# lastdancewithyou/multimodal_edema_prediction

Hardware: AMD Instinct MI355X
Metric: multimodal train samples/sec (higher is better)
Workload: dtype bf16

## Files before the change

### include/medp_hip.h

```cpp
#ifndef MEDP_HIP_H
#define MEDP_HIP_H
#include <stddef.h>

#ifdef __cplusplus
extern "C" {
#endif

const char* medp_last_error(void);
int medp_version(void);
const char* medp_arch(void);

int medp_gemm_bf16_nt(const void* A, const void* W, void* C, int M, int N, int K, int lda, int ldw, int ldc,
                      const float* bias, const float* scale, const float* residual, int ldr, int act, int out_bf16,
                      void* stream);

size_t medp_gemm_nt_workspace_bytes(int M, int N, int K);
int medp_gemm_bf16_nt_ws(const void* A, const void* W, void* C, int M, int N, int K, int lda, int ldw, int ldc, const float* bias,
                         const float* scale, const float* residual, int ldr, int act, int out_bf16, float* workspace,
                         size_t workspace_bytes, void* stream);

int medp_gemm_f32_nt(const float* A, const float* W, float* C, int M, int N, int K, int lda, int ldw, int ldc, const float* bias,
                     const float* scale, const float* residual, int ldr, int act, void* stream);
int medp_gemm_f32_tn(const float* dY, const float* X, float* C, int M, int N, int K, int lddy, int ldx, void* stream);

size_t medp_gemm_tn_workspace_bytes(int M, int N, int K);
int medp_gemm_bf16_tn(const void* dY, const void* X, float* C, int M, int N, int K, int lddy, int ldx, float* workspace, void* stream);

int medp_gemm_persistent_cap(int cap);

int medp_gemm_profile_enable(int mode);
int medp_gemm_profile_collect(double* host_total_ms, long long* host_n_launches, double* host_total_flops);

int medp_attn_fwd_dh64(const void* q, const void* k, const void* v, void* o, int B, int S, int H, int ldq, int ldk,
                       int ldv, int ldo, float scale, void* stream);
int medp_attn_dh16_fwd(const float* qkv, int ld, void* o_bf16, int ldo, int B, int N, int H, int dh, float scale, void* stream);
int medp_attn_dh16_train_supported(int B, int N, int H, int dh, int ld, int ldo);
int medp_attn_dh16_train_fwd(const void* qkv, int ld, void* o, int ldo, float* lse, int io_bf16, int B, int N, int H, int dh, float scale,
                             float dropout_p, unsigned seed, unsigned stream_id, void* stream);
int medp_attn_dh16_train_bwd(const void* dout, int lddo, const void* qkv, int ld, const float* lse, float* delta_ws, void* dqkv,
                             int lddqkv, int io_bf16, int B, int N, int H, int dh, float scale, float dropout_p, unsigned seed,
                             unsigned stream_id, void* stream);
int medp_attn_fwd_dh64_lse(const void* q, const void* k, const void* v, void* o, float* lse, int B, int S, int H, int ldq,
                           int ldk, int ldv, int ldo, float scale, void* stream);
int medp_attn_bwd_dh64_prep(const float* dout, int lddout, const void* o_bf16, int ldo, void* dout_bf16, int lddob,
                            float* dsum, int B, int S, int H, void* stream);
int medp_attn_bwd_dh64(const void* q, const void* k, const void* v, int ldqkv, const void* dout_bf16, int lddo,
                       const float* lse, const float* dsum, float* dq, float* dk, float* dv, int ldd, int B, int S, int H,
                       float scale, void* stream);
int medp_attn_small_fwd(const float* q, int ldq, long long q_batch_stride, const float* k, const float* v, int ldkv,
                        long long kv_batch_stride, void* o, int ldo, int o_bf16, float* attn_avg, int B, int Lq, int Lk,
                        int H, int dh, float scale, float dropout_p, unsigned seed, unsigned stream_id, void* stream);
int medp_attn_small_bwd(const float* dout, int lddo, const float* q, int ldq, long long q_batch_stride, const float* k,
                        const float* v, int ldkv, long long kv_batch_stride, float* dq, int lddq, float* dk, int lddkv,
                        float* dv, int reserved, long long dkv_batch_stride, int B, int Lq, int Lk, int H, int dh, float scale,
                        float dropout_p, unsigned seed, unsigned stream_id, void* stream);
int medp_attn_small_masked_fwd(const float* q, int ldq, long long q_batch_stride, const float* k, const float* v, int ldkv,
                               long long kv_batch_stride, void* o, int ldo, int o_bf16, float* attn_avg, int B, int Lq, int Lk,
                               int H, int dh, float scale, float dropout_p, unsigned seed, unsigned stream_id, void* stream,
                               const unsigned char* key_mask, long long mask_batch_stride);
int medp_attn_small_masked_bwd(const float* dout, int lddo, const float* q, int ldq, long long q_batch_stride, const float* k,
                               const float* v, int ldkv, long long kv_batch_stride, float* dq, int lddq, float* dk, int lddkv,
                               float* dv, int reserved, long long dkv_batch_stride, int B, int Lq, int Lk, int H, int dh, float scale,
                               float dropout_p, unsigned seed, unsigned stream_id, void* stream, const unsigned char* key_mask,
                               long long mask_batch_stride);

size_t medp_attn_fq_split_ws_bytes(int B, int H, int Lq, int Lk, int bwd);
int medp_attn_fq_split_fwd(const float* q, int ldq, long long q_batch_stride, const float* k, const float* v, int ldkv,
                           long long kv_batch_stride, void* o, int ldo, int o_bf16, float* lse, float* attn_avg, float* ws,
                           size_t ws_bytes, int B, int Lq, int Lk, int H, int dh, float scale, float dropout_p, unsigned seed,
                           unsigned stream_id, void* stream);
int medp_attn_fq_split_bwd(const float* dout, int lddo, const float* o, int ldo, const float* lse, const float* q, int ldq,
                           long long q_batch_stride, const float* k, const float* v, int ldkv, long long kv_batch_stride, float* dq,
                           int lddq, float* dk, float* dv, int lddkv, long long dkv_batch_stride, float* ws, size_t ws_bytes, int B,
                           int Lq, int Lk, int H, int dh, float scale, float dropout_p, unsigned seed, unsigned stream_id,
                           void* stream);

int medp_layernorm_fwd(const float* x, int ldx, const float* w, const float* b, void* y, int ldy, int y_bf16, float* mean,
                       float* rstd, int rows, int D, float eps, void* stream);
size_t medp_colsum_workspace_bytes(int rows, int D);
int medp_layernorm_bwd(const float* dy, int lddy, const float* x, int ldx, const float* w, const float* mean,
                       const float* rstd, float* dx, int lddx, int accumulate_dx, float* dw, float* db, float* workspace,
                       int rows, int D, void* stream);
int medp_colsum_f32(const float* x, int ldx, float* out, float* workspace, int rows, int D, void* stream);
int medp_scalenorm_fwd(const float* x, int ldx, const float* g, void* y, int ldy, int y_bf16, float* rnorm, int rows, int D,
                       float eps, void* stream);
int medp_scalenorm_bwd(const float* dy, int lddy, const float* x, int ldx, const float* g, const float* rnorm, float* dx,
                       int lddx, int accumulate_dx, float* dg, float* workspace_rows, int rows, int D, void* stream);
int medp_scalenorm_bwd_add(const float* dy, int lddy, const float* x, int ldx, const float* g, const float* rnorm, const float* add,
                           int ldadd, float* dx, int lddx, float* dg, float* workspace_rows, int rows, int D, void* stream);

int medp_cast_f32_bf16(const float* x, int ldx, void* y, int ldy, int rows, int cols, void* stream);
int medp_transpose_to_bf16(const void* x, int x_is_bf16, int ldx, void* y, int ldy, int rows, int cols, void* stream);
typedef struct {
    const void* src;
    void* dst_plain;
    void* dst_t;
    int rows, cols, ld_src, ld_plain, ld_t, reserved_;
} MedpOperandJob;
int medp_weight_operands_multi(const MedpOperandJob* dev_jobs, const int* dev_block_job, const int* dev_block_tile, int n_blocks,
                               void* stream);
int medp_gelu_bwd(const float* dy, const float* pre, float* dx, long long n, void* stream);
int medp_gelu_bf16_fwd(const void* pre, void* out, long long n, void* stream);
int medp_gelu_bf16_bwd(const void* dy, const void* pre, void* dx, long long n, void* stream);
int medp_im2col_patch(const float* pix, void* A, int B, int C, int H, int W, int patch, int kpad, void* stream);
int medp_vit_assemble(const float* patch, const float* cls, const float* pos, float* x, int B, int P, int D, void* stream);
int medp_pos_embed_bicubic(const float* pos, float* out, int src_side, int gh, int gw, int D, void* stream);
int medp_pos_embed_bicubic_bwd(const float* dout, float* dpos, int src_side, int gh, int gw, int D, void* stream);

typedef struct {
    const float *ln1_w, *ln1_b;
    const void* qkv_w;
    const float* qkv_b;
    const void* proj_w;
    const float *proj_b, *ls1;
    const float *ln2_w, *ln2_b;
    const void* fc1_w;
    const float* fc1_b;
    const void* fc2_w;
    const float *fc2_b, *ls2;
    const void *qkv_wg, *fc1_wg;
    const float *qkv_cs, *qkv_b2, *fc1_cs, *fc1_b2;
} MedpVitLayer;

typedef struct {
    int hidden, n_layers, n_heads, mlp_hidden, patch, pos_side, patch_kpad;
    float ln_eps;
    const void* patch_w;
    const float *patch_b, *cls, *pos;
    const float *final_ln_w, *final_ln_b;
    const MedpVitLayer* layers;
} MedpVitWeights;

size_t medp_vit_workspace_bytes(const MedpVitWeights* host_w, int B, int H, int W);
int medp_vit_forward(const MedpVitWeights* host_w, const float* pixels, int B, int H, int W, float* tokens_f32,
                     void* tokens_bf16, void* workspace, size_t workspace_bytes, void* stream);
int medp_vit_forward_part(const MedpVitWeights* w, const float* pixels, int B, int H, int W, float* tokens_f32, void* tokens_bf16,
                          void* workspace, size_t workspace_bytes, int first_layer, int last_layer, void* stream);

typedef struct {
    const float* g_attn;
    const void* qkv_w;
    const void* out_w;
    const float* g_ff;
    const void* ff1_w;
    const float* ff1_b;
    const void* ff2_w;
    const float* ff2_b;
    const float* g_final;
} MedpEncoderWeights;

typedef struct {
    int n_vars, n_static, d_embedding, n_heads, n_layers, d_ff, d_hidden_embed, d_hidden_tab, d_hidden_time, n_obs_rows,
        final_norm;
    float norm_eps;
    const void *emb_w0, *emb_b0, *emb_bn_scale, *emb_bn_shift, *emb_w4, *emb_b4;
    const void *emb_l0, *emb_w4t;
    const void* n_obs_table;
    const void *tab_w0, *tab_b0, *tab_bn_scale, *tab_bn_shift, *tab_w4, *tab_b4;
    const void* special;
    const void *time_w0, *time_b0, *time_bn_scale, *time_bn_shift, *time_w3t, *time_b3;
    const void* rep_embedding;
    const void* event_embedding;
    const MedpEncoderWeights* event_enc;
    const MedpEncoderWeights* time_enc;
} MedpDuettWeights;

int medp_duett_embed_fwd(const MedpDuettWeights* host_w, const float* xs_static, const float* xs_ts, const float* xs_times, int B, int T,
                         float* xe_out, void* h_out_bf16, float* temb_out, float* psi0_out, float* tab_workspace, int stages, void* stream);
int medp_duett_swap_add_norm(const float* in, const float* rnorm, const float* g_prev, const float* add, long long add_batch_stride,
                             const float* g_norm, float norm_eps, float* x_out, void* h_out_bf16, int B, int A1, int A2, int E,
                             void* stream);

int medp_feats_to_input(const float* const* ts_ptrs, const float* ts_base, long long ts_stride, const float* const* time_ptrs,
                        const float* time_base, long long time_stride, const int* lengths, int T_uniform, const float* static_in,
                        float* xs_ts, float* xs_times, float* xs_static, int B, int V, int Ds, int max_len, int Tpad, float aug_noise,
                        float aug_mask, unsigned seed, unsigned stream_id, void* stream);
int medp_ssl_mask_batch(const float* xs_ts, const int* mask_t, const int* event_idx, const unsigned char* keep, float* clipped,
                        float* y_ts, float* y_masks, float* y_events, float* y_events_mask, int B, int T, int V, void* stream);

size_t medp_duett_workspace_bytes(const MedpDuettWeights* host_w, int B, int T);
int medp_duett_encode(const MedpDuettWeights* host_w, const float* xs_static, const float* xs_ts, const float* xs_times, int B,
                      int T, float* tokens_f32, void* tokens_bf16, float* psi0_out, void* workspace, size_t workspace_bytes,
                      void* stream);

int medp_gelu_dropout_fwd(const float* x, float* y, long long n, float p, unsigned seed, unsigned stream_id, void* stream);
int medp_gelu_dropout_bwd(const float* dy, const float* x, float* dx, long long n, float p, unsigned seed, unsigned stream_id,
                          void* stream);
int medp_gelu_dropout_fwd_bf16(const float* x, void* y_bf16, long long n, float p, unsigned seed, unsigned stream_id, void* stream);
int medp_gelu_dropout_bwd_bf16(const float* dy, const float* x, float* dx, void* dx_bf16, long long n, float p, unsigned seed,
                               unsigned stream_id, void* stream);
int medp_dropout_add(const float* y, const float* residual, float* out, long long n, float p, unsigned seed, unsigned stream_id,
                     void* stream);
int medp_rowdot_fwd(const float* x, int ldx, const float* w, const float* b, float* y, int rows, int D, void* stream);
int medp_rowdot_bwd(const float* dy, const float* x, int ldx, const float* w, float* dx, float* dw, float* db, int rows, int D,
                    void* stream);
int medp_fusion_logits_fwd(const float* hi, const float* ht, const float* hc, const float* img_bias, const float* ts_bias,
                           const float* beta, float* img, float* ts, float* scaled, float* fus, int B, int K, void* stream);
int medp_fusion_logits_bwd(const float* d_img, const float* d_ts, const float* d_scaled, const float* d_fus, const float* hc,
                           const float* beta, float* d_hi, float* d_ht, float* d_hc, float* d_img_bias, float* d_ts_bias,
                           float* d_beta, int B, int K, void* stream);
int medp_meanpool_fwd(const float* x, float* y, int B, int T, int T1, int D, void* stream);
int medp_meanpool_bwd(const float* dy, float* dx, int B, int T, int T1, int D, void* stream);

int medp_dual_pathology_loss(const float* img, const float* ts, const float* fus, const float* y, const float* mask,
                             const float* label_weights, const float* pos_weight, float alpha_img, float alpha_ts,
                             float alpha_fus, float eps, float* out, float* g_img, float* g_ts, float* g_fus, int B, int K,
                             void* stream);
int medp_student_kd_loss(const float* z_s, const float* z_t, const float* y, float T, float alpha, float pos_weight, float* out,
                         float* g_zs, int B, void* stream);

int medp_aux_residual_kl(const float* img_logits, const float* scaled_correction, const float* y, const float* mask,
                         float label_smoothing, float* out, float* g_scaled, int n, void* stream);
int medp_sq_mean(const float* x, float coef, float* out, float* g, int n, void* stream);
int medp_masked_bce_global(const float* logits, const float* y, const float* mask, float* out, float* g, int n, void* stream);

int medp_masked_mse(const float* a, const float* b, const float* mask, float* out, float* g_a, int n, void* stream);
int medp_bce_mean(const float* logits, const float* y, const float* weight, float* out, float* g, int n, void* stream);

typedef struct {
    void* param;
    const void* grad;
    void* exp_avg;
    void* exp_avg_sq;
    long long numel;
    float lr, weight_decay;
} MedpAdamTensor;
int medp_adamw_chunk_elems(void);
int medp_adamw_multi(const MedpAdamTensor* dev_descs, const int* dev_block_tensor, const int* dev_block_chunk, int n_blocks,
                     float beta1, float beta2, float eps, int step, const unsigned* dev_step, float grad_scale, void* stream);
int medp_grad_sumsq_multi(const MedpAdamTensor* dev_descs, const int* dev_block_tensor, const int* dev_block_chunk, int n_blocks,
                          float* dev_partials, float max_norm, float* dev_out, void* stream);
int medp_adamw_multi_dscale(const MedpAdamTensor* dev_descs, const int* dev_block_tensor, const int* dev_block_chunk, int n_blocks,
                            float beta1, float beta2, float eps, int step, const unsigned* dev_step, const float* dev_grad_scale,
                            void* stream);

int medp_rng_set_epoch_ptr(const unsigned* dev_ptr);
int medp_counter_advance(unsigned* dev_counter, void* stream);

int medp_glinear_fwd(const float* x, const float* W, const float* b, float* y, int G, int R, int K, int N, void* stream);
size_t medp_glinear_bwd_workspace_bytes(int G, int R, int K, int N);
int medp_glinear_bwd(const float* dy, const float* x, const float* W, float* dx, float* dW, float* db, float* workspace, int G, int R,
                     int K, int N, void* stream);
int medp_gmlp_supported(int KIN, int C, int E);
size_t medp_gmlp_workspace_bytes(int G, int R, int KIN, int C, int E);
int medp_gmlp_fwd(const float* x, const float* W0, const float* b0, const float* bn_w, const float* bn_b, float* running_mean,
                  float* running_var, const float* W1, const float* b1, float* out, float* save_mean, float* save_var, int G, int R,
                  int KIN, int C, int E, float eps, float momentum, int batch_stats, float* workspace, void* stream);
int medp_gmlp_bwd(const float* dout, const float* x, const float* W0, const float* b0, const float* bn_w, const float* bn_b,
                  const float* save_mean, const float* save_var, const float* W1, float* dx, float* dW0, float* db0, float* dbn_w,
                  float* dbn_b, float* dW1, float* db1, int G, int R, int KIN, int C, int E, float eps, int batch_stats,
                  float* workspace, void* stream);
size_t medp_gbn_workspace_bytes(int G, int R, int C);
int medp_gbn_fwd(const float* x, const float* w, const float* b, float* running_mean, float* running_var, float* y, float* save_mean,
                 float* save_var, int G, int R, int C, float eps, float momentum, int batch_stats, float* workspace, void* stream);
int medp_gbn_bwd(const float* dy, const float* x, const float* w, const float* save_mean, const float* save_var, float* dx, float* dw,
                 float* db, int G, int R, int C, float eps, int batch_stats, float* workspace, void* stream);
int medp_act_fwd(const float* x, float* y, long long n, int mode , void* stream);
int medp_act_bwd(const float* dy, const float* y, float* dx, long long n, int mode, void* stream);
int medp_embed_inputs_fwd(const float* xs_ts, const float* n_obs_table, int table_rows, float* xin, int B, int T, int V, int KP,
                          void* stream);
int medp_embed_inputs_bwd_blocks(int B, int T, int V);
int medp_embed_inputs_bwd(const float* xs_ts, const float* d_xin, float* partial, int table_rows, int B, int T, int V, int KP,
                          void* stream);
int medp_psi_assemble_fwd(const float* xs_ts, const float* var_out, const float* tab_out, const float* special, float* psi, int B, int T,
                          int V, int E, void* stream);
int medp_psi_assemble_bwd_slices(int B, int T, int V);
int medp_psi_assemble_bwd(const float* xs_ts, const float* dpsi, float* d_var_out, float* d_tab_partial, float* d_special_partial, int B,
                          int T, int V, int E, void* stream);
int medp_axis_swap(const float* in, float* out, int B, int A1, int A2, int E, void* stream);
int medp_axis_swap_add(const float* in, const float* add, const float* add_last, float* out, int B, int A1, int A2, int E, int mode,
                       void* stream);
int medp_add_bcast(const float* a, const float* b, float* out, long long per_batch, int B, int broadcast_b, void* stream);

int medp_traj_features(const float* x, float* out, int B, int T, int V, void* stream);
int medp_gru_fwd(const float* gi, const void* whh_bf16, const float* bhh, float* hseq, float* gates, float* hn, int S, int T, int d,
                 void* stream);
int medp_gru_fwd_f32(const float* gi, const float* whh_t, int ld_whh_t, const float* bhh, float* hseq, float* gates, float* hn, int S,
                     int T, int d, void* stream);
int medp_gru_bwd(const float* dh, const float* gates, const float* hn, const float* hseq, const void* whh_t_bf16, float* dgi,
                 float* dghn, void* dgh_bf16, int S, int T, int d, void* stream);

#ifdef __cplusplus
}
#endif
#endif
```

### multimodal_edema_prediction_amd/abi.py

```python
from __future__ import annotations

import ctypes
import os
from ctypes import c_char_p, c_float, c_int, c_longlong, c_size_t, c_uint, c_void_p

import torch

_HERE = os.path.dirname(os.path.abspath(__file__))
LIB_PATH = os.environ.get("MEDP_HIP_LIB") or os.path.join(_HERE, "libmedp_hip.so")

P, I, F, U, LL, SZ = c_void_p, c_int, c_float, c_uint, c_longlong, c_size_t


class MedpVitLayer(ctypes.Structure):
    _fields_ = [(n, P) for n in ("ln1_w", "ln1_b", "qkv_w", "qkv_b", "proj_w", "proj_b", "ls1", "ln2_w", "ln2_b",
                                 "fc1_w", "fc1_b", "fc2_w", "fc2_b", "ls2",
                                 "qkv_wg", "fc1_wg", "qkv_cs", "qkv_b2", "fc1_cs", "fc1_b2")]


class MedpVitWeights(ctypes.Structure):
    _fields_ = ([(n, I) for n in ("hidden", "n_layers", "n_heads", "mlp_hidden", "patch", "pos_side", "patch_kpad")]
                + [("ln_eps", F)]
                + [(n, P) for n in ("patch_w", "patch_b", "cls", "pos", "final_ln_w", "final_ln_b")]
                + [("layers", ctypes.POINTER(MedpVitLayer))])


class MedpEncoderWeights(ctypes.Structure):
    _fields_ = [(n, P) for n in ("g_attn", "qkv_w", "out_w", "g_ff", "ff1_w", "ff1_b", "ff2_w", "ff2_b", "g_final")]


class MedpDuettWeights(ctypes.Structure):
    _fields_ = ([(n, I) for n in ("n_vars", "n_static", "d_embedding", "n_heads", "n_layers", "d_ff", "d_hidden_embed",
                                  "d_hidden_tab", "d_hidden_time", "n_obs_rows", "final_norm")]
                + [("norm_eps", F)]
                + [(n, P) for n in ("emb_w0", "emb_b0", "emb_bn_scale", "emb_bn_shift", "emb_w4", "emb_b4", "emb_l0", "emb_w4t", "n_obs_table",
                                    "tab_w0", "tab_b0", "tab_bn_scale", "tab_bn_shift", "tab_w4", "tab_b4", "special",
                                    "time_w0", "time_b0", "time_bn_scale", "time_bn_shift", "time_w3t", "time_b3",
                                    "rep_embedding", "event_embedding")]
                + [("event_enc", ctypes.POINTER(MedpEncoderWeights)), ("time_enc", ctypes.POINTER(MedpEncoderWeights))])


class MedpAdamTensor(ctypes.Structure):
    _fields_ = [("param", P), ("grad", P), ("exp_avg", P), ("exp_avg_sq", P), ("numel", LL), ("lr", F), ("weight_decay", F)]


class MedpOperandJob(ctypes.Structure):
    _fields_ = [("src", P), ("dst_plain", P), ("dst_t", P), ("rows", I), ("cols", I), ("ld_src", I), ("ld_plain", I), ("ld_t", I),
                ("reserved_", I)]


SIGNATURES = {
    "medp_last_error": (c_char_p, []),
    "medp_version": (I, []),
    "medp_arch": (c_char_p, []),
    "medp_gemm_bf16_nt": (I, [P, P, P, I, I, I, I, I, I, P, P, P, I, I, I, P]),
    "medp_gemm_nt_workspace_bytes": (SZ, [I, I, I]),
    "medp_gemm_bf16_nt_ws": (I, [P, P, P, I, I, I, I, I, I, P, P, P, I, I, I, P, SZ, P]),
    "medp_gemm_f32_nt": (I, [P, P, P, I, I, I, I, I, I, P, P, P, I, I, P]),
    "medp_gemm_f32_tn": (I, [P, P, P, I, I, I, I, I, P]),
    "medp_gemm_tn_workspace_bytes": (SZ, [I, I, I]),
    "medp_gemm_bf16_tn": (I, [P, P, P, I, I, I, I, I, P, P]),
    "medp_gemm_persistent_cap": (I, [I]),
    "medp_gemm_profile_enable": (I, [I]),
    "medp_gemm_profile_collect": (I, [ctypes.POINTER(ctypes.c_double), ctypes.POINTER(c_longlong), ctypes.POINTER(ctypes.c_double)]),
    "medp_attn_fwd_dh64": (I, [P, P, P, P, I, I, I, I, I, I, I, F, P]),
    "medp_attn_dh16_fwd": (I, [P, I, P, I, I, I, I, I, F, P]),
    "medp_attn_dh16_train_supported": (I, [I, I, I, I, I, I]),
    "medp_attn_dh16_train_fwd": (I, [P, I, P, I, P, I, I, I, I, I, F, F, U, U, P]),
    "medp_attn_dh16_train_bwd": (I, [P, I, P, I, P, P, P, I, I, I, I, I, I, F, F, U, U, P]),
    "medp_attn_fwd_dh64_lse": (I, [P, P, P, P, P, I, I, I, I, I, I, I, F, P]),
    "medp_attn_bwd_dh64_prep": (I, [P, I, P, I, P, I, P, I, I, I, P]),
    "medp_attn_bwd_dh64": (I, [P, P, P, I, P, I, P, P, P, P, P, I, I, I, I, F, P]),
    "medp_attn_small_fwd": (I, [P, I, LL, P, P, I, LL, P, I, I, P, I, I, I, I, I, F, F, U, U, P]),
    "medp_attn_small_bwd": (I, [P, I, P, I, LL, P, P, I, LL, P, I, P, I, P, I, LL, I, I, I, I, I, F, F, U, U, P]),
    "medp_attn_small_masked_fwd": (I, [P, I, LL, P, P, I, LL, P, I, I, P, I, I, I, I, I, F, F, U, U, P, P, LL]),
    "medp_attn_small_masked_bwd": (I, [P, I, P, I, LL, P, P, I, LL, P, I, P, I, P, I, LL, I, I, I, I, I, F, F, U, U, P, P, LL]),
    "medp_attn_fq_split_ws_bytes": (SZ, [I, I, I, I, I]),
    "medp_attn_fq_split_fwd": (I, [P, I, LL, P, P, I, LL, P, I, I, P, P, P, SZ, I, I, I, I, I, F, F, U, U, P]),
    "medp_attn_fq_split_bwd": (I, [P, I, P, I, P, P, I, LL, P, P, I, LL, P, I, P, P, I, LL, P, SZ, I, I, I, I, I, F, F, U, U, P]),
    "medp_layernorm_fwd": (I, [P, I, P, P, P, I, I, P, P, I, I, F, P]),
    "medp_colsum_workspace_bytes": (SZ, [I, I]),
    "medp_layernorm_bwd": (I, [P, I, P, I, P, P, P, P, I, I, P, P, P, I, I, P]),
    "medp_colsum_f32": (I, [P, I, P, P, I, I, P]),
    "medp_scalenorm_fwd": (I, [P, I, P, P, I, I, P, I, I, F, P]),
    "medp_scalenorm_bwd": (I, [P, I, P, I, P, P, P, I, I, P, P, I, I, P]),
    "medp_scalenorm_bwd_add": (I, [P, I, P, I, P, P, P, I, P, I, P, P, I, I, P]),
    "medp_cast_f32_bf16": (I, [P, I, P, I, I, I, P]),
    "medp_transpose_to_bf16": (I, [P, I, I, P, I, I, I, P]),
    "medp_weight_operands_multi": (I, [P, P, P, I, P]),
    "medp_gelu_bwd": (I, [P, P, P, LL, P]),
    "medp_gelu_bf16_fwd": (I, [P, P, LL, P]),
    "medp_gelu_bf16_bwd": (I, [P, P, P, LL, P]),
    "medp_im2col_patch": (I, [P, P, I, I, I, I, I, I, P]),
    "medp_vit_assemble": (I, [P, P, P, P, I, I, I, P]),
    "medp_pos_embed_bicubic": (I, [P, P, I, I, I, I, P]),
    "medp_pos_embed_bicubic_bwd": (I, [P, P, I, I, I, I, P]),
    "medp_vit_workspace_bytes": (SZ, [ctypes.POINTER(MedpVitWeights), I, I, I]),
    "medp_vit_forward": (I, [ctypes.POINTER(MedpVitWeights), P, I, I, I, P, P, P, SZ, P]),
    "medp_vit_forward_part": (I, [ctypes.POINTER(MedpVitWeights), P, I, I, I, P, P, P, SZ, I, I, P]),
    "medp_duett_embed_fwd": (I, [ctypes.POINTER(MedpDuettWeights), P, P, P, I, I, P, P, P, P, P, I, P]),
    "medp_duett_swap_add_norm": (I, [P, P, P, P, LL, P, F, P, P, I, I, I, I, P]),
    "medp_feats_to_input": (I, [P, P, LL, P, P, LL, P, I, P, P, P, P, I, I, I, I, I, F, F, U, U, P]),
    "medp_ssl_mask_batch": (I, [P, P, P, P, P, P, P, P, P, I, I, I, P]),
    "medp_duett_workspace_bytes": (SZ, [ctypes.POINTER(MedpDuettWeights), I, I]),
    "medp_duett_encode": (I, [ctypes.POINTER(MedpDuettWeights), P, P, P, I, I, P, P, P, P, SZ, P]),
    "medp_gelu_dropout_fwd": (I, [P, P, LL, F, U, U, P]),
    "medp_gelu_dropout_bwd": (I, [P, P, P, LL, F, U, U, P]),
    "medp_gelu_dropout_fwd_bf16": (I, [P, P, LL, F, U, U, P]),
    "medp_gelu_dropout_bwd_bf16": (I, [P, P, P, P, LL, F, U, U, P]),
    "medp_dropout_add": (I, [P, P, P, LL, F, U, U, P]),
    "medp_rowdot_fwd": (I, [P, I, P, P, P, I, I, P]),
    "medp_rowdot_bwd": (I, [P, P, I, P, P, P, P, I, I, P]),
    "medp_fusion_logits_fwd": (I, [P, P, P, P, P, P, P, P, P, P, I, I, P]),
    "medp_fusion_logits_bwd": (I, [P, P, P, P, P, P, P, P, P, P, P, P, I, I, P]),
    "medp_meanpool_fwd": (I, [P, P, I, I, I, I, P]),
    "medp_meanpool_bwd": (I, [P, P, I, I, I, I, P]),
    "medp_dual_pathology_loss": (I, [P, P, P, P, P, P, P, F, F, F, F, P, P, P, P, I, I, P]),
    "medp_student_kd_loss": (I, [P, P, P, F, F, F, P, P, I, P]),
    "medp_aux_residual_kl": (I, [P, P, P, P, F, P, P, I, P]),
    "medp_sq_mean": (I, [P, F, P, P, I, P]),
    "medp_masked_bce_global": (I, [P, P, P, P, P, I, P]),
    "medp_glinear_fwd": (I, [P, P, P, P, I, I, I, I, P]),
    "medp_glinear_bwd_workspace_bytes": (SZ, [I, I, I, I]),
    "medp_glinear_bwd": (I, [P, P, P, P, P, P, P, I, I, I, I, P]),
    "medp_gmlp_supported": (I, [I, I, I]),
    "medp_gmlp_workspace_bytes": (SZ, [I, I, I, I, I]),
    "medp_gmlp_fwd": (I, [P] * 12 + [I, I, I, I, I, F, F, I, P, P]),
    "medp_gmlp_bwd": (I, [P] * 16 + [I, I, I, I, I, F, I, P, P]),
    "medp_gbn_workspace_bytes": (SZ, [I, I, I]),
    "medp_gbn_fwd": (I, [P, P, P, P, P, P, P, P, I, I, I, F, F, I, P, P]),
    "medp_gbn_bwd": (I, [P, P, P, P, P, P, P, P, I, I, I, F, I, P, P]),
    "medp_act_fwd": (I, [P, P, LL, I, P]),
    "medp_act_bwd": (I, [P, P, P, LL, I, P]),
    "medp_embed_inputs_fwd": (I, [P, P, I, P, I, I, I, I, P]),
    "medp_embed_inputs_bwd_blocks": (I, [I, I, I]),
    "medp_embed_inputs_bwd": (I, [P, P, P, I, I, I, I, I, P]),
    "medp_psi_assemble_fwd": (I, [P, P, P, P, P, I, I, I, I, P]),
    "medp_psi_assemble_bwd_slices": (I, [I, I, I]),
    "medp_psi_assemble_bwd": (I, [P, P, P, P, P, I, I, I, I, P]),
    "medp_axis_swap": (I, [P, P, I, I, I, I, P]),
    "medp_axis_swap_add": (I, [P, P, P, P, I, I, I, I, I, P]),
    "medp_add_bcast": (I, [P, P, P, LL, I, I, P]),
    "medp_masked_mse": (I, [P, P, P, P, P, I, P]),
    "medp_bce_mean": (I, [P, P, P, P, P, I, P]),
    "medp_adamw_chunk_elems": (I, []),
    "medp_adamw_multi": (I, [P, P, P, I, F, F, F, I, P, F, P]),
    "medp_grad_sumsq_multi": (I, [P, P, P, I, P, F, P, P]),
    "medp_adamw_multi_dscale": (I, [P, P, P, I, F, F, F, I, P, P, P]),
    "medp_traj_features": (I, [P, P, I, I, I, P]),
    "medp_gru_fwd": (I, [P, P, P, P, P, P, I, I, I, P]),
    "medp_gru_fwd_f32": (I, [P, P, I, P, P, P, P, I, I, I, P]),
    "medp_gru_bwd": (I, [P, P, P, P, P, P, P, P, I, I, I, P]),
    "medp_rng_set_epoch_ptr": (I, [P]),
    "medp_counter_advance": (I, [P, P]),
}

_lib = None


def lib() -> ctypes.CDLL:
    global _lib
    if _lib is None:
        if not os.path.exists(LIB_PATH):
            raise RuntimeError(
                f"HIP extension {LIB_PATH} is missing: build it with `python -m multimodal_edema_prediction_amd.build` "
                "(hipcc --offload-arch=gfx950). There is no CPU fallback for the hot path.")
        L = ctypes.CDLL(LIB_PATH)
        for name, (res, args) in SIGNATURES.items():
            fn = getattr(L, name)
            fn.restype, fn.argtypes = res, args
        _lib = L
    return _lib


def check(rc: int, what: str = "") -> None:
    if rc == 0:
        return
    msg = lib().medp_last_error().decode("utf-8", "replace")
    if rc < 0:
        raise ValueError(f"{what}: {msg}" if what else msg)
    raise RuntimeError(f"{what}: HIP error {rc}: {msg}")


def stream() -> int:
    return torch.cuda.current_stream().cuda_stream


def ptr(t: torch.Tensor | None) -> int | None:
    if t is None:
        return None
    if not t.is_cuda:
        raise RuntimeError("libmedp_hip operates on GPU memory only (tensor is on %s); there is no CPU fallback" % t.device)
    return t.data_ptr()


def require_gpu() -> None:
    lib()
    if not torch.cuda.is_available():
        raise RuntimeError("no HIP device is visible: the MI355X hot path cannot run (there is no CPU fallback)")
```

### multimodal_edema_prediction_amd/csrc/api.cpp

```cpp
#include <stdarg.h>
#include <stdio.h>

#include "medp_hip.h"

static thread_local char g_err[512] = "";

void medp_set_error(const char* fmt, ...) {
    va_list ap;
    va_start(ap, fmt);
    vsnprintf(g_err, sizeof(g_err), fmt, ap);
    va_end(ap);
}

extern "C" const char* medp_last_error(void) { return g_err; }
extern "C" int medp_version(void) { return 2; }
extern "C" const char* medp_arch(void) { return "gfx950"; }

#include <stdint.h>
static const uint32_t* g_rng_epoch = nullptr;
const uint32_t* medp_rng_epoch_ptr() { return g_rng_epoch; }
extern "C" int medp_rng_set_epoch_ptr(const unsigned* dev_ptr) {
    g_rng_epoch = dev_ptr;
    return 0;
}
```

### multimodal_edema_prediction_amd/csrc/elementwise.hip

```cpp
#include "common.h"
#include "medp_hip.h"

namespace {

__global__ __launch_bounds__(256) void cast_f32_bf16_kernel(const float* __restrict__ x, int ldx, bf16_t* __restrict__ y, int ldy,
                                                            int rows, int cols) {
    const int c4 = cols >> 2;
    const size_t total = (size_t)rows * c4;
    for (size_t i = (size_t)blockIdx.x * 256 + threadIdx.x; i < total; i += (size_t)gridDim.x * 256) {
        const int r = (int)(i / c4), c = (int)(i % c4) * 4;
        const float4 v = *(const float4*)(x + (size_t)r * ldx + c);
        uint2 o;
        o.x = pack_bf2(v.x, v.y);
        o.y = pack_bf2(v.z, v.w);
        *(uint2*)(y + (size_t)r * ldy + c) = o;
    }
}

template <typename TIN>
__global__ __launch_bounds__(256) void transpose_to_bf16_kernel(const TIN* __restrict__ x, int ldx, bf16_t* __restrict__ y, int ldy,
                                                                int rows, int cols) {
    __shared__ float tile[64][65];
    const int r0 = blockIdx.y * 64, c0 = blockIdx.x * 64;
    const int tx = threadIdx.x & 63, ty = threadIdx.x >> 6;
    for (int i = ty; i < 64; i += 4) {
        const int r = r0 + i, c = c0 + tx;
        float v = 0.f;
        if (r < rows && c < cols) {
            if constexpr (sizeof(TIN) == 2) v = bf2f(((const bf16_t*)x)[(size_t)r * ldx + c]);
            else v = ((const float*)x)[(size_t)r * ldx + c];
        }
        tile[i][tx] = v;
    }
    __syncthreads();
    for (int i = ty; i < 64; i += 4) {
        const int c = c0 + i, r = r0 + tx;
        if (c < cols && r < rows) y[(size_t)c * ldy + r] = f2bf(tile[tx][i]);
    }
}

__global__ __launch_bounds__(256) void weight_operands_multi_kernel(const MedpOperandJob* __restrict__ jobs, const int* __restrict__ blk_job,
                                                                    const int* __restrict__ blk_tile) {
    __shared__ float tile[64][65];
    const MedpOperandJob j = jobs[blk_job[blockIdx.x]];
    const int tiles_c = (j.cols + 63) / 64;
    const int t = blk_tile[blockIdx.x];
    const int r0 = (t / tiles_c) * 64, c0 = (t % tiles_c) * 64;
    const int tx = threadIdx.x & 63, ty = threadIdx.x >> 6;
    const float* x = (const float*)j.src;
    bf16_t* yp = (bf16_t*)j.dst_plain;
    bf16_t* yt = (bf16_t*)j.dst_t;
    for (int i = ty; i < 64; i += 4) {
        const int r = r0 + i, c = c0 + tx;
        float v = 0.f;
        if (r < j.rows && c < j.cols) {
            v = x[(size_t)r * j.ld_src + c];
            if (yp) yp[(size_t)r * j.ld_plain + c] = f2bf(v);
        }
        tile[i][tx] = v;
    }
    if (!yt) return;
    __syncthreads();
    for (int i = ty; i < 64; i += 4) {
        const int c = c0 + i, r = r0 + tx;
        if (c < j.cols && r < j.rows) yt[(size_t)c * j.ld_t + r] = f2bf(tile[tx][i]);
    }
}

__global__ __launch_bounds__(256) void gelu_bwd_kernel(const float* __restrict__ dy, const float* __restrict__ pre, float* __restrict__ dx,
                                                       size_t n) {
    for (size_t i = ((size_t)blockIdx.x * 256 + threadIdx.x) * 4; i < n; i += (size_t)gridDim.x * 1024) {
        const float4 g = *(const float4*)(dy + i), p = *(const float4*)(pre + i);
        *(float4*)(dx + i) = make_float4(g.x * gelu_erf_grad(p.x), g.y * gelu_erf_grad(p.y), g.z * gelu_erf_grad(p.z),
                                         g.w * gelu_erf_grad(p.w));
    }
}

__global__ __launch_bounds__(256) void gelu_bf16_fwd_kernel(const bf16_t* __restrict__ pre, bf16_t* __restrict__ out, size_t n8) {
    for (size_t i = (size_t)blockIdx.x * 256 + threadIdx.x; i < n8; i += (size_t)gridDim.x * 256) {
        const uint4 p = *(const uint4*)(pre + i * 8);
        const uint32_t w[4] = {p.x, p.y, p.z, p.w};
        uint32_t o[4];
#pragma unroll
        for (int k = 0; k < 4; ++k) {
            const f32x2 g = gelu_erf2((f32x2){__uint_as_float(w[k] << 16), __uint_as_float(w[k] & 0xffff0000u)});
            o[k] = pack_bf2(g[0], g[1]);
        }
        *(uint4*)(out + i * 8) = make_uint4(o[0], o[1], o[2], o[3]);
    }
}
__global__ __launch_bounds__(256) void gelu_bf16_bwd_kernel(const bf16_t* __restrict__ dy, const bf16_t* __restrict__ pre,
                                                            bf16_t* __restrict__ dx, size_t n8) {
    for (size_t i = (size_t)blockIdx.x * 256 + threadIdx.x; i < n8; i += (size_t)gridDim.x * 256) {
        const uint4 g = *(const uint4*)(dy + i * 8), p = *(const uint4*)(pre + i * 8);
        const uint32_t gw[4] = {g.x, g.y, g.z, g.w}, pw[4] = {p.x, p.y, p.z, p.w};
        uint32_t o[4];
#pragma unroll
        for (int k = 0; k < 4; ++k) {
            const float a = __uint_as_float(gw[k] << 16) * gelu_erf_grad(__uint_as_float(pw[k] << 16));
            const float b = __uint_as_float(gw[k] & 0xffff0000u) * gelu_erf_grad(__uint_as_float(pw[k] & 0xffff0000u));
            o[k] = pack_bf2(a, b);
        }
        *(uint4*)(dx + i * 8) = make_uint4(o[0], o[1], o[2], o[3]);
    }
}

__global__ __launch_bounds__(256) void im2col_patch_kernel(const float* __restrict__ pix, bf16_t* __restrict__ A, int B, int C, int H,
                                                           int W, int ps, int kpad) {
    const unsigned gh = H / ps, gw = W / ps, K = C * ps * ps, pp = ps * ps, k8 = kpad >> 3;
    const unsigned total = (unsigned)B * gh * gw * k8;
    for (unsigned i = blockIdx.x * 256u + threadIdx.x; i < total; i += gridDim.x * 256u) {
        const unsigned kc = i % k8, row = i / k8;
        const unsigned px = row % gw, r2 = row / gw, py = r2 % gh, b = r2 / gh;
        const float* img = pix + (size_t)b * C * H * W + (size_t)(py * ps) * W + px * ps;
        float v[8];
#pragma unroll
        for (int u = 0; u < 8; ++u) {
            const unsigned kk = kc * 8 + u;
            float x = 0.f;
            if (kk < K) {
                const unsigned c = kk / pp, rem = kk - c * pp, ii = rem / ps, jj = rem - ii * ps;
                x = img[((size_t)c * H + ii) * W + jj];
            }
            v[u] = x;
        }
        uint4 o;
        o.x = pack_bf2(v[0], v[1]);
        o.y = pack_bf2(v[2], v[3]);
        o.z = pack_bf2(v[4], v[5]);
        o.w = pack_bf2(v[6], v[7]);
        *(uint4*)(A + (size_t)row * kpad + kc * 8) = o;
    }
}

__global__ __launch_bounds__(256) void vit_assemble_kernel(const float* __restrict__ patch, const float* __restrict__ cls,
                                                           const float* __restrict__ pos, float* __restrict__ x, int B, int P, int D) {
    const int d4 = D >> 2;
    const size_t total = (size_t)B * (P + 1) * d4;
    for (size_t i = (size_t)blockIdx.x * 256 + threadIdx.x; i < total; i += (size_t)gridDim.x * 256) {
        const int c = (int)(i % d4) * 4;
        const size_t tokrow = i / d4;
        const int t = (int)(tokrow % (P + 1)), b = (int)(tokrow / (P + 1));
        const float4 pe = *(const float4*)(pos + (size_t)t * D + c);
        const float4 v = (t == 0) ? *(const float4*)(cls + c) : *(const float4*)(patch + ((size_t)b * P + t - 1) * D + c);
        *(float4*)(x + tokrow * D + c) = make_float4(v.x + pe.x, v.y + pe.y, v.z + pe.z, v.w + pe.w);
    }
}

__device__ __forceinline__ float cubic1(float x, float A) { return ((A + 2.f) * x - (A + 3.f)) * x * x + 1.f; }
__device__ __forceinline__ float cubic2(float x, float A) { return ((A * x - 5.f * A) * x + 8.f * A) * x - 4.f * A; }
__global__ __launch_bounds__(256) void pos_bicubic_kernel(const float* __restrict__ pos, float* __restrict__ out, int s, int gh, int gw,
                                                          int D) {
    const size_t total = (size_t)(gh * gw + 1) * D;
    const float A = -0.75f;
    for (size_t i = (size_t)blockIdx.x * 256 + threadIdx.x; i < total; i += (size_t)gridDim.x * 256) {
        const int d = (int)(i % D), t = (int)(i / D);
        if (t == 0) { out[i] = pos[d]; continue; }
        const int oy = (t - 1) / gw, ox = (t - 1) % gw;
        const float sy = (float)s / (float)gh, sx = (float)s / (float)gw;
        const float fy = (oy + 0.5f) * sy - 0.5f, fx = (ox + 0.5f) * sx - 0.5f;
        const int iy = (int)floorf(fy), ix = (int)floorf(fx);
        const float ty = fy - iy, tx = fx - ix;
        const float wy[4] = {cubic2(ty + 1.f, A), cubic1(ty, A), cubic1(1.f - ty, A), cubic2(2.f - ty, A)};
        const float wx[4] = {cubic2(tx + 1.f, A), cubic1(tx, A), cubic1(1.f - tx, A), cubic2(2.f - tx, A)};
        float acc = 0.f;
#pragma unroll
        for (int a = 0; a < 4; ++a) {
            const int yy = min(max(iy - 1 + a, 0), s - 1);
            float rowacc = 0.f;
#pragma unroll
            for (int c = 0; c < 4; ++c) {
                const int xx = min(max(ix - 1 + c, 0), s - 1);
                rowacc += wx[c] * pos[(size_t)(1 + yy * s + xx) * D + d];
            }
            acc += wy[a] * rowacc;
        }
        out[i] = acc;
    }
}

__device__ __forceinline__ float bicubic_tap_weight(int src, int dst, int s, int g) {
    const float A = -0.75f;
    const float sc = (float)s / (float)g;
    const float f = (dst + 0.5f) * sc - 0.5f;
    const int i0 = (int)floorf(f);
    const float t = f - i0;
    const float w[4] = {cubic2(t + 1.f, A), cubic1(t, A), cubic1(1.f - t, A), cubic2(2.f - t, A)};
    float acc = 0.f;
#pragma unroll
    for (int a = 0; a < 4; ++a)
        if (min(max(i0 - 1 + a, 0), s - 1) == src) acc += w[a];
    return acc;
}
__global__ __launch_bounds__(256) void pos_bicubic_bwd_kernel(const float* __restrict__ dout, float* __restrict__ dpos, int s, int gh,
                                                              int gw, int D) {
    const int d4n = D >> 2;
    const int total = (s * s + 1) * d4n;
    for (int i = blockIdx.x * 256 + threadIdx.x; i < total; i += gridDim.x * 256) {
        const int d4 = i % d4n, cell = i / d4n;
        if (cell == 0) {
            *(float4*)(dpos + 4 * d4) = *(const float4*)(dout + 4 * d4);
            continue;
        }
        const int sy = (cell - 1) / s, sx = (cell - 1) % s;
        float4 acc = make_float4(0.f, 0.f, 0.f, 0.f);
        for (int oy = 0; oy < gh; ++oy) {
            const float wy = bicubic_tap_weight(sy, oy, s, gh);
            if (wy == 0.f) continue;
            for (int ox = 0; ox < gw; ++ox) {
                const float wx = bicubic_tap_weight(sx, ox, s, gw);
                if (wx == 0.f) continue;
                const float w = wy * wx;
                const float4 g = *(const float4*)(dout + (size_t)(1 + oy * gw + ox) * D + 4 * d4);
                acc.x += w * g.x; acc.y += w * g.y; acc.z += w * g.z; acc.w += w * g.w;
            }
        }
        *(float4*)(dpos + (size_t)cell * D + 4 * d4) = acc;
    }
}

inline int grid_for(size_t work_items) { return (int)min((size_t)4096, max((size_t)1, (work_items + 255) / 256)); }

}

extern "C" int medp_cast_f32_bf16(const float* x, int ldx, void* y, int ldy, int rows, int cols, void* stream) {
    MEDP_CHECK_ARG(x && y && rows > 0 && cols > 0, "cast: bad argument");
    MEDP_CHECK_ARG(cols % 4 == 0 && ldx % 4 == 0 && ldy % 4 == 0, "cast: cols, ldx, ldy must be multiples of 4");
    cast_f32_bf16_kernel<<<grid_for((size_t)rows * cols / 4), 256, 0, (hipStream_t)stream>>>(x, ldx, (bf16_t*)y, ldy, rows, cols);
    MEDP_LAUNCH_CHECK("medp_cast_f32_bf16");
    return 0;
}

extern "C" int medp_transpose_to_bf16(const void* x, int x_is_bf16, int ldx, void* y, int ldy, int rows, int cols, void* stream) {
    MEDP_CHECK_ARG(x && y && rows > 0 && cols > 0 && ldx >= cols && ldy >= rows, "transpose: bad argument");
    dim3 grid((cols + 63) / 64, (rows + 63) / 64);
    if (x_is_bf16)
        transpose_to_bf16_kernel<bf16_t><<<grid, 256, 0, (hipStream_t)stream>>>((const bf16_t*)x, ldx, (bf16_t*)y, ldy, rows, cols);
    else
        transpose_to_bf16_kernel<float><<<grid, 256, 0, (hipStream_t)stream>>>((const float*)x, ldx, (bf16_t*)y, ldy, rows, cols);
    MEDP_LAUNCH_CHECK("medp_transpose_to_bf16");
    return 0;
}

extern "C" int medp_weight_operands_multi(const MedpOperandJob* dev_jobs, const int* dev_block_job, const int* dev_block_tile, int n_blocks,
                                          void* stream) {
    MEDP_CHECK_ARG(dev_jobs && dev_block_job && dev_block_tile && n_blocks > 0, "weight_operands_multi: bad argument");
    weight_operands_multi_kernel<<<n_blocks, 256, 0, (hipStream_t)stream>>>(dev_jobs, dev_block_job, dev_block_tile);
    MEDP_LAUNCH_CHECK("medp_weight_operands_multi");
    return 0;
}

extern "C" int medp_gelu_bwd(const float* dy, const float* pre, float* dx, long long n, void* stream) {
    MEDP_CHECK_ARG(dy && pre && dx && n > 0 && n % 4 == 0, "gelu_bwd: bad argument (n must be a multiple of 4)");
    gelu_bwd_kernel<<<grid_for((size_t)n / 4), 256, 0, (hipStream_t)stream>>>(dy, pre, dx, (size_t)n);
    MEDP_LAUNCH_CHECK("medp_gelu_bwd");
    return 0;
}

extern "C" int medp_gelu_bf16_fwd(const void* pre, void* out, long long n, void* stream) {
    MEDP_CHECK_ARG(pre && out && n > 0 && n % 8 == 0, "gelu_bf16_fwd: bad argument (n must be a multiple of 8)");
    gelu_bf16_fwd_kernel<<<grid_for((size_t)n / 8), 256, 0, (hipStream_t)stream>>>((const bf16_t*)pre, (bf16_t*)out, (size_t)n / 8);
    MEDP_LAUNCH_CHECK("medp_gelu_bf16_fwd");
    return 0;
}

extern "C" int medp_gelu_bf16_bwd(const void* dy, const void* pre, void* dx, long long n, void* stream) {
    MEDP_CHECK_ARG(dy && pre && dx && n > 0 && n % 8 == 0, "gelu_bf16_bwd: bad argument (n must be a multiple of 8)");
    gelu_bf16_bwd_kernel<<<grid_for((size_t)n / 8), 256, 0, (hipStream_t)stream>>>((const bf16_t*)dy, (const bf16_t*)pre, (bf16_t*)dx,
                                                                                  (size_t)n / 8);
    MEDP_LAUNCH_CHECK("medp_gelu_bf16_bwd");
    return 0;
}

extern "C" int medp_im2col_patch(const float* pix, void* A, int B, int C, int H, int W, int patch, int kpad, void* stream) {
    MEDP_CHECK_ARG(pix && A && B > 0 && C > 0 && patch > 0, "im2col: bad argument");
    MEDP_CHECK_ARG(H >= patch && W >= patch, "im2col: image %dx%d smaller than the patch size %d", H, W, patch);
    MEDP_CHECK_ARG(kpad >= C * patch * patch && kpad % 8 == 0, "im2col: kpad must be >= C*p*p and a multiple of 8");
    const size_t total = (size_t)B * (H / patch) * (W / patch) * (kpad / 8);
    MEDP_CHECK_ARG(total < (1ull << 31), "im2col: B * patches * kpad / 8 must stay below 2^31");
    im2col_patch_kernel<<<grid_for(total), 256, 0, (hipStream_t)stream>>>(pix, (bf16_t*)A, B, C, H, W, patch, kpad);
    MEDP_LAUNCH_CHECK("medp_im2col_patch");
    return 0;
}

extern "C" int medp_vit_assemble(const float* patch, const float* cls, const float* pos, float* x, int B, int P, int D, void* stream) {
    MEDP_CHECK_ARG(patch && cls && pos && x && B > 0 && P > 0 && D % 4 == 0, "vit_assemble: bad argument");
    vit_assemble_kernel<<<grid_for((size_t)B * (P + 1) * D / 4), 256, 0, (hipStream_t)stream>>>(patch, cls, pos, x, B, P, D);
    MEDP_LAUNCH_CHECK("medp_vit_assemble");
    return 0;
}

extern "C" int medp_pos_embed_bicubic_bwd(const float* dout, float* dpos, int src_side, int gh, int gw, int D, void* stream) {
    MEDP_CHECK_ARG(dout && dpos && src_side > 0 && gh > 0 && gw > 0 && D > 0 && D % 4 == 0, "pos_embed_bicubic_bwd: bad argument");
    pos_bicubic_bwd_kernel<<<grid_for((size_t)(src_side * src_side + 1) * (D / 4)), 256, 0, (hipStream_t)stream>>>(dout, dpos, src_side, gh, gw, D);
    MEDP_LAUNCH_CHECK("medp_pos_embed_bicubic_bwd");
    return 0;
}

extern "C" int medp_pos_embed_bicubic(const float* pos, float* out, int src_side, int gh, int gw, int D, void* stream) {
    MEDP_CHECK_ARG(pos && out && src_side > 0 && gh > 0 && gw > 0 && D > 0, "pos_embed_bicubic: bad argument");
    pos_bicubic_kernel<<<grid_for((size_t)(gh * gw + 1) * D), 256, 0, (hipStream_t)stream>>>(pos, out, src_side, gh, gw, D);
    MEDP_LAUNCH_CHECK("medp_pos_embed_bicubic");
    return 0;
}
```

### multimodal_edema_prediction_amd/csrc/gemm_bf16.hip

```cpp
#include <stdlib.h>

#include <vector>

#include <algorithm>

#include "common.h"
#include "gemm_variants.h"
#include "medp_hip.h"

namespace {

__device__ __attribute__((aligned(16))) uint32_t g_zero16[4] = {0, 0, 0, 0};

struct GemmParams {
    const bf16_t* A;
    const bf16_t* W;
    void* C;
    int M, N, K, lda, ldw, ldc;
    const float* bias;
    const float* scale;
    const float* residual;
    int ldr;
    int act;
    int out_bf16;
    float* partial;
    int nsplit;
};

__device__ __forceinline__ void glds16(const void* gsrc, void* lds_wave_base) {
    __builtin_amdgcn_global_load_lds((const __attribute__((address_space(1))) void*)gsrc,
                                     (__attribute__((address_space(3))) void*)lds_wave_base, 16, 0, 0);
}

template <int BM, int BN, int TAG>
__global__ __launch_bounds__(256, 2) void gemm_bf16_nt_kernel(const GemmParams p) {
    extern __shared__ __attribute__((aligned(16))) char smem[];
    constexpr int A_BYTES = BM * 128, B_BYTES = BN * 128, STAGE = A_BYTES + B_BYTES;
    constexpr int TM = BM / 32, TN = BN / 32;

    const int tid = threadIdx.x, lane = tid & 63;
    const int wave = __builtin_amdgcn_readfirstlane(tid >> 6);
    const int fr = lane & 15, kq = lane >> 4;
    const int wr = wave >> 1, wc = wave & 1;

    const int tiles_n = (p.N + BN - 1) / BN, tiles_m = (p.M + BM - 1) / BM;
    const int nwg = tiles_m * tiles_n;
    const int bid = blockIdx.x;
    const int q = nwg >> 3, r = nwg & 7, xcd = bid & 7;
    const int wg = (xcd < r ? xcd * (q + 1) : r * (q + 1) + (xcd - r) * q) + (bid >> 3);
    const int m0 = (wg / tiles_n) * BM, n0 = (wg % tiles_n) * BN;

    const int nkt_all = (p.K + 63) >> 6;
    const int per_split = (nkt_all + p.nsplit - 1) / p.nsplit;
    const int kt_begin = blockIdx.y * per_split;
    const int nkt = max(0, min(nkt_all, kt_begin + per_split) - kt_begin);
    const bf16_t* zero = (const bf16_t*)g_zero16;

    auto stage = [&](int buf, int kt) {
        char* sa = smem + buf * STAGE;
        char* sb = sa + A_BYTES;
        const int k0 = (kt_begin + kt) << 6;
#pragma unroll
        for (int i = 0; i < BM * 8 / 256; ++i) {
            const int qd = i * 256 + tid;
            const int row = qd >> 3, c = (qd & 7) ^ (row & 7);
            const int gr = m0 + row, gk = k0 + c * 8;
            const bf16_t* src = (gr < p.M && gk < p.K) ? p.A + (size_t)gr * p.lda + gk : zero;
            glds16(src, sa + (i * 256 + wave * 64) * 16);
        }
#pragma unroll
        for (int i = 0; i < BN * 8 / 256; ++i) {
            const int qd = i * 256 + tid;
            const int row = qd >> 3, c = (qd & 7) ^ (row & 7);
            const int gr = n0 + row, gk = k0 + c * 8;
            const bf16_t* src = (gr < p.N && gk < p.K) ? p.W + (size_t)gr * p.ldw + gk : zero;
            glds16(src, sb + (i * 256 + wave * 64) * 16);
        }
    };

    f32x4 acc[TM][TN];
#pragma unroll
    for (int i = 0; i < TM; ++i)
#pragma unroll
        for (int j = 0; j < TN; ++j) acc[i][j] = (f32x4){0.f, 0.f, 0.f, 0.f};

    if (nkt > 0) stage(0, 0);
    MEDP_WAIT_LDS_DMA();
    __syncthreads();

    const int a_row0 = wr * (BM / 2) + fr, b_row0 = wc * (BN / 2) + fr;
    const int sw = fr & 7;

    for (int kt = 0; kt < nkt; ++kt) {
        const int cur = kt & 1;
        if (kt + 1 < nkt) stage(cur ^ 1, kt + 1);
        const char* sa = smem + cur * STAGE;
        const char* sb = sa + A_BYTES;
#pragma unroll
        for (int s = 0; s < 2; ++s) {
            const int coff = ((s * 4 + kq) ^ sw) << 4;
            bf16x8 xa[TM], wb[TN];
#pragma unroll
            for (int i = 0; i < TM; ++i) xa[i] = *(const bf16x8*)(sa + (a_row0 + i * 16) * 128 + coff);
#pragma unroll
            for (int j = 0; j < TN; ++j) wb[j] = *(const bf16x8*)(sb + (b_row0 + j * 16) * 128 + coff);
#pragma unroll
            for (int i = 0; i < TM; ++i)
#pragma unroll
                for (int j = 0; j < TN; ++j)
                    acc[i][j] = __builtin_amdgcn_mfma_f32_16x16x32_bf16(wb[j], xa[i], acc[i][j], 0, 0, 0);
        }
        MEDP_WAIT_LDS_DMA();
        __syncthreads();
    }

#pragma unroll
    for (int i = 0; i < TM; ++i) {
        const int m = m0 + wr * (BM / 2) + i * 16 + fr;
        if (m >= p.M) continue;
#pragma unroll
        for (int j = 0; j < TN; ++j) {
            const int n = n0 + wc * (BN / 2) + j * 16 + kq * 4;
            if (n >= p.N) continue;
            f32x4 v = acc[i][j];
            if (p.partial) {
                *(f32x4*)(p.partial + ((size_t)blockIdx.y * p.M + m) * p.N + n) = v;
                continue;
            }
            if (p.bias) {
                const f32x4 b = *(const f32x4*)(p.bias + n);
                v += b;
            }
            if (p.act == 1) {
                    v = gelu_erf4(v);
            }
            if (p.scale) {
                const f32x4 sc = *(const f32x4*)(p.scale + n);
                v *= sc;
            }
            if (p.residual) {
                const f32x4 rs = *(const f32x4*)(p.residual + (size_t)m * p.ldr + n);
                v += rs;
            }
            if (p.out_bf16) {
                uint2 o;
                o.x = pack_bf2(v[0], v[1]);
                o.y = pack_bf2(v[2], v[3]);
                *(uint2*)((bf16_t*)p.C + (size_t)m * p.ldc + n) = o;
            } else {
                *(f32x4*)((float*)p.C + (size_t)m * p.ldc + n) = v;
            }
        }
    }
}


template <int TAG>
__global__ __launch_bounds__(256, 2) void gemm_bf16_nt_v3_kernel(const GemmParams p) {
    extern __shared__ __attribute__((aligned(16))) char smem[];
    constexpr int BM = 256, BN = 128;
    constexpr int A_BYTES = BM * 64, B_BYTES = BN * 64, STAGE = A_BYTES + B_BYTES;

    const int tid = threadIdx.x, lane = tid & 63;
    const int wave = __builtin_amdgcn_readfirstlane(tid >> 6);
    const int fr = lane & 15, kq = lane >> 4;
    const int wm = wave >> 1, wn = wave & 1;

    const int tiles_n = (p.N + BN - 1) / BN, tiles_m = (p.M + BM - 1) / BM;
    const int nwg = tiles_m * tiles_n;
    const int bid = blockIdx.x;
    const int q = nwg >> 3, r = nwg & 7, xcd = bid & 7;
    const int wg = (xcd < r ? xcd * (q + 1) : r * (q + 1) + (xcd - r) * q) + (bid >> 3);
    constexpr int MB = 8, SN = 8;
    const int band = wg / (MB * tiles_n), rb = wg % (MB * tiles_n);
    const int mb = min(MB, tiles_m - band * MB);
    const int sc = rb / (mb * SN), r2 = rb % (mb * SN);
    const int sn = min(SN, tiles_n - sc * SN);
    const int m0 = (band * MB + r2 / sn) * BM, n0 = (sc * SN + r2 % sn) * BN;
    const int nkt = (p.K + 31) >> 5;
    const bf16_t* zero = (const bf16_t*)g_zero16;

    auto stage_piece = [&](int slot, int kt, int piece) {
        char* sa = smem + slot * STAGE;
        const int k0 = kt << 5;
        if (piece < 4) {
            const int qd = piece * 256 + tid;
            const int row = qd >> 2, c = (qd & 3) ^ (((row >> 2) & 1) << 1);
            const int gr = m0 + row, gk = k0 + c * 8;
            const bf16_t* src = (gr < p.M && gk < p.K) ? p.A + (size_t)gr * p.lda + gk : zero;
            glds16(src, sa + (piece * 256 + wave * 64) * 16);
        } else {
            const int qd = (piece - 4) * 256 + tid;
            const int row = qd >> 2, c = (qd & 3) ^ (((row >> 2) & 1) << 1);
            const int gr = n0 + row, gk = k0 + c * 8;
            const bf16_t* src = (gr < p.N && gk < p.K) ? p.W + (size_t)gr * p.ldw + gk : zero;
            glds16(src, sa + A_BYTES + ((piece - 4) * 256 + wave * 64) * 16);
        }
    };

    f32x4 acc[8][4];
#pragma unroll
    for (int i = 0; i < 8; ++i)
#pragma unroll
        for (int j = 0; j < 4; ++j) acc[i][j] = (f32x4){0.f, 0.f, 0.f, 0.f};

#pragma unroll
    for (int pc = 0; pc < 6; ++pc) stage_piece(0, 0, pc);
#pragma unroll
    for (int pc = 0; pc < 6; ++pc) stage_piece(1, 1, pc);

    const int coff = (kq ^ (((fr >> 2) & 1) << 1)) << 4;
    const int a_off = (wm * 128 + fr) * 64 + coff, b_off = (wn * 64 + fr) * 64 + coff;
    int slot = 0;
    for (int kt = 0; kt < nkt; ++kt) {
        asm volatile("s_waitcnt vmcnt(6)" ::: "memory");
        __builtin_amdgcn_s_barrier();
        const char* sa = smem + slot * STAGE + a_off;
        const char* sb = smem + slot * STAGE + A_BYTES + b_off;
        const int nslot = slot == 0 ? 2 : slot - 1;
        bf16x8 xa[8], wb[4];
#pragma unroll
        for (int j = 0; j < 4; ++j) wb[j] = *(const bf16x8*)(sb + j * 16 * 64);
#pragma unroll
        for (int i = 0; i < 8; ++i) xa[i] = *(const bf16x8*)(sa + i * 16 * 64);
#pragma unroll
        for (int i = 0; i < 8; ++i) {
#pragma unroll
            for (int j = 0; j < 4; ++j)
                acc[i][j] = __builtin_amdgcn_mfma_f32_16x16x32_bf16(wb[j], xa[i], acc[i][j], 0, 0, 0);
            if (i < 6) stage_piece(nslot, kt + 2, i);
        }
        __builtin_amdgcn_sched_group_barrier(0x100, 6, 0);
#pragma unroll
        for (int g = 0; g < 6; ++g) {
            __builtin_amdgcn_sched_group_barrier(0x008, 4, 0);
            __builtin_amdgcn_sched_group_barrier(0x100, 1, 0);
        }
        __builtin_amdgcn_sched_group_barrier(0x008, 8, 0);
        slot = slot == 2 ? 0 : slot + 1;
    }

    asm volatile("s_waitcnt vmcnt(0)" ::: "memory");
    __syncthreads();
    float* wl = (float*)(smem + wave * (64 * 68 * 4));
    const int er = lane >> 4, ec = (lane & 15) * 4;
    const int n = n0 + wn * 64 + ec;
    f32x4 bias4 = (f32x4){0.f, 0.f, 0.f, 0.f}, scale4 = (f32x4){1.f, 1.f, 1.f, 1.f};
    if (n < p.N) {
        if (p.bias) bias4 = *(const f32x4*)(p.bias + n);
        if (p.scale) scale4 = *(const f32x4*)(p.scale + n);
    }
#pragma unroll
    for (int half = 0; half < 2; ++half) {
#pragma unroll
        for (int i4 = 0; i4 < 4; ++i4)
#pragma unroll
            for (int j = 0; j < 4; ++j) *(f32x4*)(wl + (i4 * 16 + fr) * 68 + j * 16 + kq * 4) = acc[half * 4 + i4][j];
        __builtin_amdgcn_fence(__ATOMIC_RELEASE, "workgroup");
        __builtin_amdgcn_wave_barrier();
        __builtin_amdgcn_fence(__ATOMIC_ACQUIRE, "workgroup");
#pragma unroll 4
        for (int it = 0; it < 16; ++it) {
            const int rr = it * 4 + er;
            const int m = m0 + wm * 128 + half * 64 + rr;
            f32x4 v = *(const f32x4*)(wl + rr * 68 + ec);
            if (m < p.M && n < p.N) {
                v += bias4;
                if (p.act == 1) {
                    v = gelu_erf4(v);
                }
                v *= scale4;
                if (p.residual) v += *(const f32x4*)(p.residual + (size_t)m * p.ldr + n);
                if (p.out_bf16) {
                    uint2 o;
                    o.x = pack_bf2(v[0], v[1]);
                    o.y = pack_bf2(v[2], v[3]);
                    *(uint2*)((bf16_t*)p.C + (size_t)m * p.ldc + n) = o;
                } else {
                    *(f32x4*)((float*)p.C + (size_t)m * p.ldc + n) = v;
                }
            }
        }
        __builtin_amdgcn_fence(__ATOMIC_RELEASE, "workgroup");
        __builtin_amdgcn_wave_barrier();
        __builtin_amdgcn_fence(__ATOMIC_ACQUIRE, "workgroup");
    }
}

__global__ __launch_bounds__(256) void splitk_finish_kernel(const GemmParams p) {
    const int n4 = p.N >> 2;
    const size_t total = (size_t)p.M * n4;
    for (size_t i = (size_t)blockIdx.x * 256 + threadIdx.x; i < total; i += (size_t)gridDim.x * 256) {
        const int m = (int)(i / n4), n = (int)(i % n4) * 4;
        f32x4 v = *(const f32x4*)(p.partial + (size_t)m * p.N + n);
        for (int s = 1; s < p.nsplit; ++s) v += *(const f32x4*)(p.partial + ((size_t)s * p.M + m) * p.N + n);
        if (p.bias) v += *(const f32x4*)(p.bias + n);
        if (p.act == 1) v = gelu_erf4(v);
        if (p.scale) v *= *(const f32x4*)(p.scale + n);
        if (p.residual) v += *(const f32x4*)(p.residual + (size_t)m * p.ldr + n);
        if (p.out_bf16) {
            uint2 o;
            o.x = pack_bf2(v[0], v[1]);
            o.y = pack_bf2(v[2], v[3]);
            *(uint2*)((bf16_t*)p.C + (size_t)m * p.ldc + n) = o;
        } else {
            *(f32x4*)((float*)p.C + (size_t)m * p.ldc + n) = v;
        }
    }
}

template <int TAG>
int launch_v3(const GemmParams& p, hipStream_t stream) {
    const int tiles = ((p.M + 255) / 256) * ((p.N + 127) / 128);
    constexpr int LDS = 3 * (256 + 128) * 64;
    MEDP_ONCE_PER_DEVICE({
        hipFuncSetAttribute((const void*)gemm_bf16_nt_v3_kernel<TAG>, hipFuncAttributeMaxDynamicSharedMemorySize, LDS);
    });
    gemm_bf16_nt_v3_kernel<TAG><<<tiles, 256, LDS, stream>>>(p);
    MEDP_LAUNCH_CHECK("medp_gemm_bf16_nt(v3)");
    return 0;
}

template <int BM, int BN, int TAG>
int launch(const GemmParams& p, hipStream_t stream) {
    const int tiles = ((p.M + BM - 1) / BM) * ((p.N + BN - 1) / BN);
    constexpr int LDS = 2 * (BM + BN) * 128;
    MEDP_ONCE_PER_DEVICE({
        hipFuncSetAttribute((const void*)gemm_bf16_nt_kernel<BM, BN, TAG>, hipFuncAttributeMaxDynamicSharedMemorySize, LDS);
    });
    gemm_bf16_nt_kernel<BM, BN, TAG><<<dim3(tiles, p.nsplit), 256, LDS, stream>>>(p);
    MEDP_LAUNCH_CHECK("medp_gemm_bf16_nt");
    if (p.partial) {
        const size_t items = (size_t)p.M * (p.N >> 2);
        splitk_finish_kernel<<<(int)min((size_t)2048, (items + 255) / 256), 256, 0, stream>>>(p);
        MEDP_LAUNCH_CHECK("medp_gemm_bf16_nt(split-K finish)");
    }
    return 0;
}

}

namespace {
struct GemmProfile {
    int mode = 0;
    int collect_mode = 0;
    std::vector<hipEvent_t> ev;
    size_t used = 0;
    double flops = 0.0;
    unsigned long long* slots = nullptr;
    std::vector<double> slot_flops;
    int slot_dev = -1;
};
constexpr size_t MAX_PROF_SLOTS = 4096;
GemmProfile g_prof;
}

extern "C" int medp_gemm_profile_enable(int mode) {
    MEDP_CHECK_ARG(mode >= 0 && mode <= 2, "gemm_profile_enable: mode must be 0 (off), 1 (HIP events) or 2 (in-kernel clock)");
    if (mode == 1) {
        g_prof.used = 0;
        g_prof.flops = 0.0;
    }
    if (mode == 2) {
        int dev = 0;
        (void)hipGetDevice(&dev);
        if (!g_prof.slots || g_prof.slot_dev != dev) {
            hipError_t e = hipMalloc((void**)&g_prof.slots, MAX_PROF_SLOTS * 4 * sizeof(unsigned long long));
            if (e != hipSuccess) { medp_set_error("gemm_profile_enable: %s", hipGetErrorString(e)); return (int)e; }
            g_prof.slot_dev = dev;
        }
        hipError_t e = hipMemset(g_prof.slots, 0, MAX_PROF_SLOTS * 4 * sizeof(unsigned long long));
        if (e != hipSuccess) { medp_set_error("gemm_profile_enable: %s", hipGetErrorString(e)); return (int)e; }
        g_prof.slot_flops.clear();
    }
    g_prof.mode = mode;
    if (mode != 0) g_prof.collect_mode = mode;
    return 0;
}

extern "C" int medp_gemm_profile_collect(double* total_ms, long long* n_launches, double* total_flops) {
    MEDP_CHECK_ARG(total_ms && n_launches && total_flops, "gemm_profile_collect: null argument");
    double ms = 0.0;
    if (g_prof.collect_mode == 2) {
        const size_t n = g_prof.slot_flops.size();
        std::vector<unsigned long long> h(n * 4);
        hipError_t e = hipMemcpy(h.data(), g_prof.slots, n * 4 * sizeof(unsigned long long), hipMemcpyDeviceToHost);
        if (e != hipSuccess) { medp_set_error("gemm_profile_collect: %s", hipGetErrorString(e)); return (int)e; }
        int khz = 100000;
        (void)hipDeviceGetAttribute(&khz, hipDeviceAttributeWallClockRate, g_prof.slot_dev);
        double fl = 0.0;
        long long cnt = 0;
        for (size_t i = 0; i < n; ++i) {
            if (h[4 * i + 1] <= h[4 * i]) continue;
            ms += (double)(h[4 * i + 1] - h[4 * i]) / (double)khz;
            fl += g_prof.slot_flops[i];
            ++cnt;
        }
        *total_ms = ms;
        *n_launches = cnt;
        *total_flops = fl;
        return 0;
    }
    for (size_t i = 0; i + 1 < g_prof.used; i += 2) {
        hipError_t e = hipEventSynchronize(g_prof.ev[i + 1]);
        if (e != hipSuccess) { medp_set_error("gemm_profile_collect: %s", hipGetErrorString(e)); return (int)e; }
        float t = 0.f;
        e = hipEventElapsedTime(&t, g_prof.ev[i], g_prof.ev[i + 1]);
        if (e != hipSuccess) { medp_set_error("gemm_profile_collect: %s", hipGetErrorString(e)); return (int)e; }
        ms += t;
    }
    *total_ms = ms;
    *n_launches = (long long)(g_prof.used / 2);
    *total_flops = g_prof.flops;
    g_prof.used = 0;
    g_prof.flops = 0.0;
    return 0;
}

extern "C" int medp_dbg_gemm_profile_raw(unsigned long long* out, int max_slots, int* n_slots, int* khz) {
    const int n = (int)std::min(g_prof.slot_flops.size(), (size_t)std::max(max_slots, 0));
    std::vector<unsigned long long> h((size_t)n * 4);
    if (n > 0 && hipMemcpy(h.data(), g_prof.slots, (size_t)n * 4 * sizeof(unsigned long long), hipMemcpyDeviceToHost) != hipSuccess) return 1;
    for (int i = 0; i < n; ++i) { out[2 * i] = h[4 * i]; out[2 * i + 1] = h[4 * i + 1]; }
    *n_slots = n;
    *khz = 100000;
    (void)hipDeviceGetAttribute(khz, hipDeviceAttributeWallClockRate, g_prof.slot_dev);
    return 0;
}

static int splitk_slices(int M, int N, int K) {
    static const int force = [] { const char* e = getenv("MEDP_GEMM_SPLITK"); return e ? atoi(e) : -1; }();
    const int tiles = ((M + 127) / 128) * (N <= 64 ? (N + 63) / 64 : (N + 127) / 128);
    const int nkt = (K + 63) / 64;
    if (force >= 0) return max(1, min(force, nkt));
    if (tiles >= 128 || nkt < 8) return 1;
    if (tiles < 64) return max(1, min(min(256 / tiles, nkt / 4), 16));
    return nkt >= 32 ? max(1, min(384 / tiles, nkt / 8)) : 1;
}

extern "C" size_t medp_gemm_nt_workspace_bytes(int M, int N, int K) {
    if (M <= 0 || N <= 0 || K <= 0) return 0;
    const int S = splitk_slices(M, N, K);
    return S > 1 ? (size_t)S * M * N * sizeof(float) : 0;
}

static int gemm_dispatch(int tag, const void* A, const void* W, void* C, int M, int N, int K, int lda, int ldw, int ldc,
                         const float* bias, const float* scale, const float* residual, int ldr, int act, int out_bf16,
                         float* workspace, size_t workspace_bytes, const MedpGemmFold* fold, void* stream);

int medp_gemm_bf16_nt_tagged_ws(int tag, const void* A, const void* W, void* C, int M, int N, int K, int lda, int ldw, int ldc,
                                const float* bias, const float* scale, const float* residual, int ldr, int act, int out_bf16,
                                float* workspace, size_t workspace_bytes, void* stream) {
    return gemm_dispatch(tag, A, W, C, M, N, K, lda, ldw, ldc, bias, scale, residual, ldr, act, out_bf16, workspace, workspace_bytes, nullptr, stream);
}

static bool uses_tile256(int M, int N) {
    static const int force = [] { const char* e = getenv("MEDP_GEMM_VARIANT"); return e ? atoi(e) : 0; }();
    const int tiles256 = ((M + 255) / 256) * ((N + 255) / 256);
    return M >= 2048 && N >= 256 && (force == 6 || (force == 0 && tiles256 >= 160));
}

bool medp_gemm_fold_eligible(int M, int N, int K) {
    static const int ragged_on = [] { const char* e = getenv("MEDP_GEMM_RAGGED"); return e ? atoi(e) : 0; }();
    return uses_tile256(M, N) && !ragged_on && K % 64 == 0 && N % 256 == 0;
}

int medp_gemm_bf16_nt_fold(const void* A, const void* W, void* C, int M, int N, int K, int lda, int ldw, int ldc, const float* bias,
                           const float* scale, const float* residual, int ldr, int act, int out_bf16, const MedpGemmFold& fold, void* stream) {
    MEDP_CHECK_ARG(medp_gemm_fold_eligible(M, N, K), "gemm(fold): M=%d N=%d K=%d does not take the 256-tile kernels", M, N, K);
    MEDP_CHECK_ARG(!fold.stats_in || (fold.colsum && fold.ln_dim > 0 && fold.stats_tiles > 0 && fold.stats_tiles <= 4 && out_bf16 && !residual && !scale),
                   "gemm(fold): a consumer needs colsum, ln_dim, 1..4 stats tiles, a bf16 result and no residual / scale");
    MEDP_CHECK_ARG(!fold.c2 || (fold.stats_out && !out_bf16 && fold.ldc2 % 4 == 0), "gemm(fold): a producer writes fp32 C, c2 (ld % 4 == 0) and stats_out");
    return gemm_dispatch(1, A, W, C, M, N, K, lda, ldw, ldc, bias, scale, residual, ldr, act, out_bf16, nullptr, 0, &fold, stream);
}

int medp_gemm_bf16_nt_tagged(int tag, const void* A, const void* W, void* C, int M, int N, int K, int lda, int ldw, int ldc,
                             const float* bias, const float* scale, const float* residual, int ldr, int act, int out_bf16,
                             void* stream) {
    return medp_gemm_bf16_nt_tagged_ws(tag, A, W, C, M, N, K, lda, ldw, ldc, bias, scale, residual, ldr, act, out_bf16, nullptr, 0, stream);
}

static int gemm_dispatch(int tag, const void* A, const void* W, void* C, int M, int N, int K, int lda, int ldw, int ldc,
                         const float* bias, const float* scale, const float* residual, int ldr, int act, int out_bf16,
                         float* workspace, size_t workspace_bytes, const MedpGemmFold* fold, void* stream) {
    MEDP_CHECK_ARG(A && W && C, "gemm: null operand");
    MEDP_CHECK_ARG(M > 0 && N > 0 && K > 0, "gemm: bad shape M=%d N=%d K=%d", M, N, K);
    MEDP_CHECK_ARG(K % 8 == 0 && lda % 8 == 0 && ldw % 8 == 0, "gemm: K, lda, ldw must be multiples of 8 (16-B chunks)");
    MEDP_CHECK_ARG(N % 4 == 0 && ldc % 4 == 0, "gemm: N and ldc must be multiples of 4 (vector epilogue)");
    MEDP_CHECK_ARG(lda >= K && ldw >= K && ldc >= N, "gemm: leading dimension smaller than the row");
    MEDP_CHECK_ARG(!residual || ldr % 4 == 0, "gemm: ldr must be a multiple of 4");
    MEDP_CHECK_ARG(((uintptr_t)A & 15) == 0 && ((uintptr_t)W & 15) == 0 && ((uintptr_t)C & 15) == 0,
                   "gemm: operands must be 16-byte aligned");
    MEDP_CHECK_ARG(act == 0 || act == 1, "gemm: act must be 0 (none) or 1 (gelu)");
    GemmParams p{(const bf16_t*)A, (const bf16_t*)W, C, M, N, K, lda, ldw, ldc, bias, scale, residual, ldr, act, out_bf16, nullptr, 1};
    hipStream_t s = (hipStream_t)stream;
    if (workspace && tag != 1) {
        const int S = splitk_slices(M, N, K);
        if (S > 1) {
            MEDP_CHECK_ARG(workspace_bytes >= (size_t)S * M * N * sizeof(float), "gemm: split-K workspace too small (medp_gemm_nt_workspace_bytes)");
            p.partial = workspace;
            p.nsplit = S;
            return N <= 64 ? launch<128, 64, 0>(p, s) : launch<128, 128, 0>(p, s);
        }
    }
    static const int force = [] { const char* e = getenv("MEDP_GEMM_VARIANT"); return e ? atoi(e) : 0; }();
    static const int v3_min_tiles = [] { const char* e = getenv("MEDP_GEMM_V3_MIN_TILES"); return e ? atoi(e) : 192; }();
    const int tiles_v3 = ((M + 255) / 256) * ((N + 127) / 128);
    const bool use_v3 = force == 3 || (force == 0 && M >= 2048 && N >= 256 && tiles_v3 >= v3_min_tiles);
    MedpGemmArgs a4{A, W, C, M, N, K, lda, ldw, ldc, bias, scale, residual, ldr, act, out_bf16, nullptr, 0};
    if (fold) a4.fold = *fold;
    if (N <= 64) return launch<128, 64, 0>(p, s);
    const bool use_v6 = uses_tile256(M, N);
    MEDP_CHECK_ARG(!fold || use_v6, "gemm(fold): shape does not take the 256-tile kernels");
    static const int v7_on = [] { const char* e = getenv("MEDP_GEMM_V7"); return e ? atoi(e) : 1; }();
    const bool use_v7 = use_v6 && force != 6 && v7_on && medp_gemm_v7_eligible(a4);
    static const int ragged_on = [] { const char* e = getenv("MEDP_GEMM_RAGGED"); return e ? atoi(e) : 0; }();
    const int rag_rows = M % 256, tiles_n256 = (N + 255) / 256, nfull256 = (M / 256) * tiles_n256;
    const bool split_ragged = use_v7 && ragged_on && rag_rows > 0 && rag_rows <= 128 && nfull256 > 256 &&
                              (nfull256 + tiles_n256 + 255) / 256 > (nfull256 + 255) / 256;
    auto launch_v67 = [&](int tg) {
        if (split_ragged) {
            MedpGemmArgs ar = a4, am = a4;
            ar.prof_flags = 2;
            am.prof_flags = 1;
            am.M = M - rag_rows;
            if (medp_gemm_v7_eligible(am)) {
                int rc = medp_gemm_ragged_rows_launch(ar, M - rag_rows, stream);
                if (rc != 0) return rc;
                rc = medp_gemm_v7_launch(am, tg, stream);
                return rc != -1 ? rc : medp_gemm_v6_launch(am, tg, stream);
            }
        }
        if (use_v7) {
            const int rc = medp_gemm_v7_launch(a4, tg, stream);
            if (rc != -1) return rc;
        }
        return medp_gemm_v6_launch(a4, tg, stream);
    };
    if (use_v6 && tag != 1) return launch_v67(0);
    if (use_v3 && tag != 1) return launch_v3<0>(p, s);
    if (tag == 1) {
        const bool prof = g_prof.mode == 1;
        if (g_prof.mode == 2 && use_v6 && g_prof.slot_flops.size() < MAX_PROF_SLOTS) {
            a4.prof = g_prof.slots + 4 * g_prof.slot_flops.size();
            g_prof.slot_flops.push_back(2.0 * (double)M * (double)N * (double)K);
        }
        if (prof) {
            if (g_prof.used + 2 > g_prof.ev.size()) {
                for (int i = 0; i < 2; ++i) {
                    hipEvent_t e;
                    if (hipEventCreate(&e) != hipSuccess) { medp_set_error("gemm profile: hipEventCreate failed"); return 1; }
                    g_prof.ev.push_back(e);
                }
            }
            hipEventRecord(g_prof.ev[g_prof.used], s);
        }
        const int rc = use_v6 ? launch_v67(1) : (use_v3 ? launch_v3<1>(p, s) : launch<128, 128, 1>(p, s));
        if (prof) {
            hipEventRecord(g_prof.ev[g_prof.used + 1], s);
            g_prof.used += 2;
            g_prof.flops += 2.0 * (double)M * (double)N * (double)K;
        }
        return rc;
    }
    return launch<128, 128, 0>(p, s);
}

extern "C" int medp_gemm_bf16_nt(const void* A, const void* W, void* C, int M, int N, int K, int lda, int ldw, int ldc,
                                 const float* bias, const float* scale, const float* residual, int ldr, int act, int out_bf16,
                                 void* stream) {
    return medp_gemm_bf16_nt_tagged(0, A, W, C, M, N, K, lda, ldw, ldc, bias, scale, residual, ldr, act, out_bf16, stream);
}

extern "C" int medp_gemm_bf16_nt_ws(const void* A, const void* W, void* C, int M, int N, int K, int lda, int ldw, int ldc,
                                    const float* bias, const float* scale, const float* residual, int ldr, int act, int out_bf16,
                                    float* workspace, size_t workspace_bytes, void* stream) {
    return medp_gemm_bf16_nt_tagged_ws(0, A, W, C, M, N, K, lda, ldw, ldc, bias, scale, residual, ldr, act, out_bf16, workspace,
                                       workspace_bytes, stream);
}
```

### multimodal_edema_prediction_amd/csrc/gemm_bf16_v6.hip

```cpp
#include <stdlib.h>

#include "common.h"
#include "gemm_tile256.h"
#include "gemm_variants.h"

namespace {

constexpr int LDS_MAIN = 2 * KBUF, LDS_EPI = 8 * 64 * 68 * 4;
constexpr int LDS_STATS = LDS_EPI;
constexpr int LDS_BYTES = LDS_STATS + 256 * 4 * 2 * 4;
static_assert(LDS_BYTES >= LDS_MAIN && LDS_BYTES <= 160 * 1024, "v6 LDS plan");

template <int TAG, int GR>
__global__ __launch_bounds__(512, 2) void gemm_bf16_nt_v6_kernel(const MedpGemmArgs p, unsigned* slot) {
    static_assert(GR == 128 || GR == 112, "v6 group rows");
    constexpr int BM = 2 * GR;
    constexpr int NI1 = (GR - 64) / 16;
    extern __shared__ __attribute__((aligned(16))) char smem[];
    const int tid = threadIdx.x, lane = tid & 63;
    const int wave = __builtin_amdgcn_readfirstlane(tid >> 6);
    const int fr = lane & 15, kq = lane >> 4;
    const int wm = wave >> 2, wn = wave & 3;
    const bf16_t* A = (const bf16_t*)p.A;
    const bf16_t* W = (const bf16_t*)p.W;
    const bf16_t* zero = (const bf16_t*)g_zero16_t256;
    MEDP_PROF_ENTER(p.prof, p.prof_flags);

    const Tile256Map map(p.M, p.N, BM);
    const int tiles_n = map.tiles_n;
    int bid = blockIdx.x;
    if (slot) {
        const int xcd = blockIdx.x & 7;
        volatile unsigned* box = (volatile unsigned*)smem;
        if (tid == 0) box[0] = __hip_atomic_fetch_add(slot + xcd, 1u, __ATOMIC_RELAXED, __HIP_MEMORY_SCOPE_AGENT);
        __syncthreads();
        bid = 8 * (int)__builtin_amdgcn_readfirstlane(box[0]) + xcd;
        __syncthreads();
        if (bid >= map.tiles_m * tiles_n) {
            if (tid == 0) {
                const unsigned left = __hip_atomic_fetch_add(slot + 8, 1u, __ATOMIC_RELAXED, __HIP_MEMORY_SCOPE_AGENT);
                if (left == gridDim.x - 1)
                    for (int i = 0; i < 9; ++i) __hip_atomic_store(slot + i, 0u, __ATOMIC_RELAXED, __HIP_MEMORY_SCOPE_AGENT);
            }
            MEDP_PROF_LEAVE(p.prof, p.prof_flags);
            return;
        }
    }
    int m0, n0;
    map.origin(bid, 8, 4, BM, m0, n0);
    const int nkt = (p.K + 63) >> 6;

    const int srow = tid >> 3, schunk = (tid & 7) ^ (srow & 7);
    const bf16_t* a_src[2][2];
    const bf16_t* w_src[2][2];
#pragma unroll
    for (int h = 0; h < 2; ++h)
#pragma unroll
        for (int j = 0; j < 2; ++j) {
            const int ra = m0 + h * GR + j * 64 + srow, rw = n0 + h * 128 + j * 64 + srow;
            a_src[h][j] = ((GR == 128 || j * 64 + srow < GR) && ra < p.M) ? A + (size_t)ra * p.lda + schunk * 8 : nullptr;
            w_src[h][j] = rw < p.N ? W + (size_t)rw * p.ldw + schunk * 8 : nullptr;
        }
    auto stage_piece = [&](int kt, int which, int j) {
        char* dst = piece_dst(smem, kt & 1, which, wave, j);
        const int k0 = kt * 64;
        const bool kin = k0 + schunk * 8 < p.K;
        const bf16_t* base = which < 2 ? a_src[which & 1][j] : w_src[which & 1][j];
        glds16((base != nullptr && kin) ? base + k0 : zero, dst);
    };
    auto stage_a = [&](int kt, int j) { stage_piece(kt, 0, j); stage_piece(kt, 1, j); };
    auto stage_w = [&](int kt, int h) { stage_piece(kt, 2 + h, 0); stage_piece(kt, 2 + h, 1); };

    f32x4 acc[8][4];
#pragma unroll
    for (int i = 0; i < 8; ++i)
#pragma unroll
        for (int j = 0; j < 4; ++j) acc[i][j] = (f32x4){0.f, 0.f, 0.f, 0.f};

    stage_a(0, 0); stage_w(0, 0); stage_w(0, 1); stage_a(0, 1);
    stage_a(1, 0); stage_w(1, 0); stage_w(1, 1);
    asm volatile("s_waitcnt vmcnt(8)" ::: "memory");

    const int sw = fr & 7;
    const int fa_off = wm * HALF + fr * 128;
    const int fw_off = 2 * HALF + (wn >> 1) * HALF + ((wn & 1) * 64 + fr) * 128;
    const int ch0 = ((0 + kq) ^ sw) << 4, ch1 = ((4 + kq) ^ sw) << 4;

    bf16x8 fa[4][2], fw0a[2][2], fw0b[2][2], fw1[2][2];
    auto read_a = [&](const char* buf, int a) {
#pragma unroll
        for (int i = 0; i < (a == 0 ? 4 : NI1); ++i) {
            const char* rp = buf + fa_off + (a * 64 + i * 16) * 128;
            fa[i][0] = *(const bf16x8*)(rp + ch0);
            fa[i][1] = *(const bf16x8*)(rp + ch1);
        }
    };
    auto read_w = [&](const char* buf, int b, bf16x8 (*fw)[2]) {
#pragma unroll
        for (int j = 0; j < 2; ++j) {
            const char* rp = buf + fw_off + (b * 32 + j * 16) * 128;
            fw[j][0] = *(const bf16x8*)(rp + ch0);
            fw[j][1] = *(const bf16x8*)(rp + ch1);
        }
    };
    const bool rows_live[2] = {m0 + wm * GR < p.M, m0 + wm * GR + 64 < p.M};
    auto mma = [&](int a, int b, const bf16x8 (*fw)[2]) {
        if (!rows_live[a]) return;
        __builtin_amdgcn_s_setprio(1);
#pragma unroll
        for (int kh = 0; kh < 2; ++kh)
#pragma unroll
            for (int i = 0; i < (a == 0 ? 4 : NI1); ++i)
#pragma unroll
                for (int j = 0; j < 2; ++j)
                    acc[a * 4 + i][b * 2 + j] = __builtin_amdgcn_mfma_f32_16x16x32_bf16(fw[j][kh], fa[i][kh], acc[a * 4 + i][b * 2 + j], 0, 0, 0);
        __builtin_amdgcn_s_setprio(0);
    };

    MEDP_BAR();
    read_w(smem, 0, fw0a);
    if (wm == 1) MEDP_BAR();

    auto none = [](int) {};
    auto ktile = [&](int kt, const bf16x8 (*fw0)[2], bf16x8 (*fw0n)[2]) {
        tile256_ktile<false>(smem, kt, fw0, fw0n, fw1, read_a, read_w, mma, stage_a, stage_w, none, none);
    };
    for (int kt = 0; kt < nkt; kt += 2) {
        ktile(kt, fw0a, fw0b);
        if (kt + 1 < nkt) ktile(kt + 1, fw0b, fw0a);
    }
    if (wm == 0) MEDP_BAR();

    asm volatile("s_waitcnt vmcnt(0)" ::: "memory");
    __syncthreads();
    float* wl = (float*)(smem + wave * (64 * 68 * 4));
    const int er = lane >> 4, ec = (lane & 15) * 4;
    const int n = n0 + wn * 64 + ec;
    f32x4 bias4 = (f32x4){0.f, 0.f, 0.f, 0.f}, scale4 = (f32x4){1.f, 1.f, 1.f, 1.f};
    if (n < p.N) {
        if (p.bias) bias4 = *(const f32x4*)(p.bias + n);
        if (p.scale) scale4 = *(const f32x4*)(p.scale + n);
    }
    f32x4 res[2][16];
    auto load_res = [&](int half) {
#pragma unroll
        for (int it = 0; it < 16; ++it) {
            const int m = m0 + wm * GR + half * 64 + it * 4 + er;
            res[half][it] = (half * 64 + it * 4 < GR && m < p.M && n < p.N) ? *(const f32x4*)(p.residual + (size_t)m * p.ldr + n) : (f32x4){0.f, 0.f, 0.f, 0.f};
        }
    };
    const bool has_res = p.residual != nullptr;
    if (has_res) load_res(0);
    const MedpGemmFold& fo = p.fold;
    const bool consumer = GR == 128 && fo.stats_in != nullptr, producer = GR == 128 && fo.c2 != nullptr;
    f32x4 cs4 = (f32x4){0.f, 0.f, 0.f, 0.f};
    if (consumer && n < p.N) cs4 = *(const f32x4*)(fo.colsum + n);
    const float inv_dim = consumer ? 1.0f / (float)fo.ln_dim : 0.f;
    float* sst = (float*)(smem + LDS_STATS);
#pragma unroll
    for (int half = 0; half < 2; ++half) {
#pragma unroll
        for (int i4 = 0; i4 < 4; ++i4)
#pragma unroll
            for (int j = 0; j < 4; ++j) *(f32x4*)(wl + (i4 * 16 + fr) * 68 + j * 16 + kq * 4) = acc[half * 4 + i4][j];
        MEDP_WAVE_LDS_SYNC();
        if (half == 0 && has_res) load_res(1);
#pragma unroll
        for (int it = 0; it < 16; ++it) {
            if (half * 64 + it * 4 >= GR) continue;
            const int rr = it * 4 + er;
            const int m = m0 + wm * GR + half * 64 + rr;
            f32x4 v = *(const f32x4*)(wl + rr * 68 + ec);
            float s1 = 0.f, s2 = 0.f;
            if (m < p.M && n < p.N) {
                if (consumer) {
                    float a1 = 0.f, a2 = 0.f;
                    for (int t = 0; t < fo.stats_tiles; ++t) {
                        const float2 st = *(const float2*)(fo.stats_in + ((size_t)m * fo.stats_tiles + t) * 2);
                        a1 += st.x;
                        a2 += st.y;
                    }
                    const float mean = a1 * inv_dim;
                    const float rstd = rsqrtf(fmaxf(a2 * inv_dim - mean * mean, 0.f) + fo.ln_eps);
                    v = v * rstd - (mean * rstd) * cs4 + bias4;
                } else {
                    v += bias4;
                }
                if (p.act == 1) v = p.out_bf16 ? gelu_bf16_4(v) : gelu_erf4(v);
                v *= scale4;
                if (has_res) v += res[half][it];
                if (p.out_bf16) {
                    uint2 o;
                    o.x = pack_bf2(v[0], v[1]);
                    o.y = pack_bf2(v[2], v[3]);
                    typedef __attribute__((ext_vector_type(2))) unsigned int u32x2;
                    __builtin_nontemporal_store((u32x2){o.x, o.y}, (u32x2*)((bf16_t*)p.C + (size_t)m * p.ldc + n));
                } else {
                    __builtin_nontemporal_store(v, (f32x4*)((float*)p.C + (size_t)m * p.ldc + n));
                }
                if (producer) {
                    uint2 o;
                    o.x = pack_bf2(v[0], v[1]);
                    o.y = pack_bf2(v[2], v[3]);
                    *(uint2*)((bf16_t*)fo.c2 + (size_t)m * fo.ldc2 + n) = o;
                    s1 = (v[0] + v[1]) + (v[2] + v[3]);
                    s2 = (v[0] * v[0] + v[1] * v[1]) + (v[2] * v[2] + v[3] * v[3]);
                }
            }
            if (producer) {
                auto row16_sum = [](float x) {
                    x += __builtin_bit_cast(float, __builtin_amdgcn_mov_dpp(__builtin_bit_cast(int, x), 0xB1, 0xF, 0xF, true));
                    x += __builtin_bit_cast(float, __builtin_amdgcn_mov_dpp(__builtin_bit_cast(int, x), 0x4E, 0xF, 0xF, true));
                    x += __builtin_bit_cast(float, __builtin_amdgcn_mov_dpp(__builtin_bit_cast(int, x), 0x141, 0xF, 0xF, true));
                    x += __builtin_bit_cast(float, __builtin_amdgcn_mov_dpp(__builtin_bit_cast(int, x), 0x140, 0xF, 0xF, true));
                    return x;
                };
                s1 = row16_sum(s1);
                s2 = row16_sum(s2);
                if ((lane & 15) == 0) *(float2*)(sst + ((wm * 128 + half * 64 + rr) * 4 + wn) * 2) = make_float2(s1, s2);
            }
        }
        MEDP_WAVE_LDS_SYNC();
    }
    if (producer) {
        __syncthreads();
        if (tid < 256 && m0 + tid < ((p.M + 255) & ~255)) {
            float a1 = 0.f, a2 = 0.f;
#pragma unroll
            for (int q = 0; q < 4; ++q) {
                const float2 st = *(const float2*)(sst + (tid * 4 + q) * 2);
                a1 += st.x;
                a2 += st.y;
            }
            *(float2*)(fo.stats_out + ((size_t)(m0 + tid) * tiles_n + n0 / BN) * 2) = make_float2(a1, a2);
        }
    }
    if (slot && tid == 0) {
        const unsigned left = __hip_atomic_fetch_add(slot + 8, 1u, __ATOMIC_RELAXED, __HIP_MEMORY_SCOPE_AGENT);
        if (left == gridDim.x - 1)
            for (int i = 0; i < 9; ++i) __hip_atomic_store(slot + i, 0u, __ATOMIC_RELAXED, __HIP_MEMORY_SCOPE_AGENT);
    }
    MEDP_PROF_LEAVE(p.prof, p.prof_flags);
}

template <int TAG, int GR>
int launch_v6_gr(const MedpGemmArgs& a, hipStream_t stream) {
    constexpr int BM = 2 * GR;
    const int tiles = ((a.M + BM - 1) / BM) * ((a.N + BN - 1) / BN);
    MEDP_ONCE_PER_DEVICE({
        hipFuncSetAttribute((const void*)gemm_bf16_nt_v6_kernel<TAG, GR>, hipFuncAttributeMaxDynamicSharedMemorySize, LDS_BYTES);
    });
    static const int tickets_on = [] { const char* e = getenv("MEDP_V6_TICKETS"); return e ? atoi(e) : 0; }();
    unsigned* slot = (tickets_on && tiles >= 64 && tiles < 256) ? medp_gemm_ticket_block(stream) : nullptr;
    gemm_bf16_nt_v6_kernel<TAG, GR><<<slot ? 256 : tiles, 512, LDS_BYTES, stream>>>(a, slot);
    MEDP_LAUNCH_CHECK("medp_gemm_bf16_nt(v6)");
    return 0;
}

bool v6_use_224(const MedpGemmArgs& a) {
    static const int mode = [] { const char* e = getenv("MEDP_V6_N768"); return e ? atoi(e) : 1; }();
    const int tiles256 = ((a.M + 255) / 256) * ((a.N + 255) / 256);
    const int tiles224 = ((a.M + 223) / 224) * ((a.N + 255) / 256);
    return mode != 0 && a.N == 768 && (a.residual != nullptr || mode == 2) && a.fold.c2 == nullptr && a.fold.stats_in == nullptr &&
           tiles256 < 256 && tiles224 <= 256;
}

}

int medp_gemm_v6_launch(const MedpGemmArgs& a, int tag, void* stream) {
    hipStream_t s = (hipStream_t)stream;
    if (v6_use_224(a)) return tag == 1 ? launch_v6_gr<1, 112>(a, s) : launch_v6_gr<0, 112>(a, s);
    return tag == 1 ? launch_v6_gr<1, 128>(a, s) : launch_v6_gr<0, 128>(a, s);
}
```

### multimodal_edema_prediction_amd/csrc/gemm_variants.h

```cpp
#pragma once
struct MedpGemmFold {
    void* c2 = nullptr;
    int ldc2 = 0;
    float* stats_out = nullptr;
    const float* stats_in = nullptr;
    int stats_tiles = 0;
    const float* colsum = nullptr;
    float ln_eps = 0.f;
    int ln_dim = 0;
};
struct MedpGemmArgs {
    const void* A;
    const void* W;
    void* C;
    int M, N, K, lda, ldw, ldc;
    const float* bias;
    const float* scale;
    const float* residual;
    int ldr, act, out_bf16;
    unsigned long long* prof;
    int prof_flags;
    MedpGemmFold fold;
};
#define MEDP_PROF_ENTER(prof, flags)                                                                                       \
    do {                                                                                                                   \
        if ((prof) && !((flags) & 1) && threadIdx.x == 0) {                                                                                \
            const unsigned long long n__ = __hip_atomic_fetch_add((prof) + 2, 1ull, __ATOMIC_RELAXED, __HIP_MEMORY_SCOPE_AGENT); \
            if (n__ % gridDim.x == 0) __hip_atomic_store((prof), wall_clock64(), __ATOMIC_RELAXED, __HIP_MEMORY_SCOPE_AGENT);   \
        }                                                                                                                  \
    } while (0)
#define MEDP_PROF_LEAVE(prof, flags)                                                                                       \
    do {                                                                                                                   \
        if ((prof) && !((flags) & 2)) {                                                                                    \
            __syncthreads();                                                                                               \
            if (threadIdx.x == 0) {                                                                                        \
                const unsigned long long n__ = __hip_atomic_fetch_add((prof) + 3, 1ull, __ATOMIC_RELAXED, __HIP_MEMORY_SCOPE_AGENT); \
                if (n__ % gridDim.x == gridDim.x - 1)                                                                      \
                    __hip_atomic_store((prof) + 1, wall_clock64(), __ATOMIC_RELAXED, __HIP_MEMORY_SCOPE_AGENT);            \
            }                                                                                                              \
        }                                                                                                                  \
    } while (0)
int medp_gemm_v6_launch(const MedpGemmArgs& a, int tag, void* stream);
int medp_gemm_ragged_rows_launch(const MedpGemmArgs& a, int m_begin, void* stream);
bool medp_gemm_v7_eligible(const MedpGemmArgs& a);
unsigned* medp_gemm_ticket_block(void* stream);
int medp_gemm_v7_launch(const MedpGemmArgs& a, int tag, void* stream);
bool medp_gemm_fold_eligible(int M, int N, int K);
int medp_gemm_bf16_nt_fold(const void* A, const void* W, void* C, int M, int N, int K, int lda, int ldw, int ldc, const float* bias,
                           const float* scale, const float* residual, int ldr, int act, int out_bf16, const MedpGemmFold& fold, void* stream);
```

### multimodal_edema_prediction_amd/csrc/vit.hip

```cpp
#include <stdlib.h>

#include "common.h"
#include "gemm_variants.h"
#include "medp_hip.h"

namespace {
inline size_t al(size_t x) { return (x + 255) & ~(size_t)255; }

struct VitWs {
    size_t a0, patch, pos, x, h, qkv, att, f, xb, stats, total;
};

template <int NT>
__global__ __launch_bounds__(256) void rowstats_cast_kernel(const float* __restrict__ x, bf16_t* __restrict__ xb, float* __restrict__ stats,
                                                            int M, int Mpad, int D) {
    const int lane = threadIdx.x & 63;
    const int row = blockIdx.x * 4 + (threadIdx.x >> 6);
    if (row >= Mpad) return;
    float s1[NT], s2[NT];
#pragma unroll
    for (int k = 0; k < NT; ++k) {
        s1[k] = s2[k] = 0.f;
        if (row < M) {
            const float4 v = *(const float4*)(x + (size_t)row * D + 4 * (lane + 64 * k));
            uint2 o;
            o.x = pack_bf2(v.x, v.y);
            o.y = pack_bf2(v.z, v.w);
            *(uint2*)(xb + (size_t)row * D + 4 * (lane + 64 * k)) = o;
            s1[k] = (v.x + v.y) + (v.z + v.w);
            s2[k] = (v.x * v.x + v.y * v.y) + (v.z * v.z + v.w * v.w);
        }
        s1[k] = wave_sum(s1[k]);
        s2[k] = wave_sum(s2[k]);
    }
    if (lane == 0) {
#pragma unroll
        for (int k = 0; k < NT; ++k) *(float2*)(stats + ((size_t)row * NT + k) * 2) = make_float2(s1[k], s2[k]);
    }
}
VitWs plan(const MedpVitWeights* w, int B, int H, int W) {
    const size_t P = (size_t)(H / w->patch) * (W / w->patch), S = P + 1, M = (size_t)B * S, D = w->hidden;
    VitWs s{};
    size_t off = 0;
    s.a0 = off;    off += al((size_t)B * P * w->patch_kpad * 2);
    s.patch = off; off += al((size_t)B * P * D * 4);
    s.pos = off;   off += al(S * D * 4);
    s.x = off;     off += al(M * D * 4);
    s.h = off;     s.att = off;  off += al(M * D * 2);
    s.qkv = off;   s.f = off;    off += al(M * (size_t)(3 * D > (size_t)w->mlp_hidden ? 3 * D : (size_t)w->mlp_hidden) * 2);
    s.xb = off;    off += al(M * D * 2);
    s.stats = off; off += al(((M + 255) / 256 * 256) * (D / 256 + 1) * 2 * 4);
    s.total = off;
    return s;
}

int g_vit_lnfold = -1;
bool fold_wanted(const MedpVitWeights* w, int M) {
    static const int env_on = [] { const char* e = getenv("MEDP_VIT_LNFOLD"); return e ? atoi(e) : 0; }();
    const int on = g_vit_lnfold >= 0 ? g_vit_lnfold : env_on;
    const int D = w->hidden;
    if (!on || D % 256 != 0 || D / 256 > 4 || w->n_layers <= 0) return false;
    for (int l = 0; l < w->n_layers; ++l) {
        const MedpVitLayer& L = w->layers[l];
        if (!L.qkv_wg || !L.fc1_wg || !L.qkv_cs || !L.qkv_b2 || !L.fc1_cs || !L.fc1_b2) return false;
    }
    return medp_gemm_fold_eligible(M, 3 * D, D) && medp_gemm_fold_eligible(M, w->mlp_hidden, D) && medp_gemm_fold_eligible(M, D, D) &&
           medp_gemm_fold_eligible(M, D, w->mlp_hidden);
}
}

extern "C" size_t medp_vit_workspace_bytes(const MedpVitWeights* w, int B, int H, int W) {
    if (!w || B <= 0 || H <= 0 || W <= 0 || w->patch <= 0) return 0;
    return plan(w, B, H, W).total;
}

extern "C" int medp_vit_forward(const MedpVitWeights* w, const float* pixels, int B, int H, int W, float* tokens_f32,
                                void* tokens_bf16, void* workspace, size_t workspace_bytes, void* stream) {
    MEDP_CHECK_ARG(w, "vit_forward: null argument");
    return medp_vit_forward_part(w, pixels, B, H, W, tokens_f32, tokens_bf16, workspace, workspace_bytes, 0, w->n_layers, stream);
}

extern "C" int medp_vit_forward_part(const MedpVitWeights* w, const float* pixels, int B, int H, int W, float* tokens_f32,
                                     void* tokens_bf16, void* workspace, size_t workspace_bytes, int first_layer, int last_layer,
                                     void* stream) {
    MEDP_CHECK_ARG(w && pixels && workspace, "vit_forward: null argument");
    MEDP_CHECK_ARG(0 <= first_layer && first_layer <= last_layer && last_layer <= w->n_layers,
                   "vit_forward: bad layer range [%d, %d) of %d", first_layer, last_layer, w->n_layers);
    const bool embed = first_layer == 0, finish = last_layer == w->n_layers;
    MEDP_CHECK_ARG(!finish || tokens_f32 || tokens_bf16, "vit_forward: no output requested");
    MEDP_CHECK_ARG(w->hidden == w->n_heads * 64, "vit_forward: head dim must be 64 (hidden %d, heads %d)", w->hidden, w->n_heads);
    MEDP_CHECK_ARG(H >= w->patch && W >= w->patch, "vit_forward: image %dx%d smaller than one patch (%d)", H, W, w->patch);
    const VitWs ws = plan(w, B, H, W);
    MEDP_CHECK_ARG(workspace_bytes >= ws.total, "vit_forward: workspace %zu < required %zu", workspace_bytes, ws.total);
    char* base = (char*)workspace;
    const int gh = H / w->patch, gw = W / w->patch, P = gh * gw, S = P + 1, M = B * S, D = w->hidden;
    void* a0 = base + ws.a0;
    float* patch = (float*)(base + ws.patch);
    float* pos = (float*)(base + ws.pos);
    float* x = (float*)(base + ws.x);
    void* h = base + ws.h;
    void* qkv = base + ws.qkv;
    void* att = base + ws.att;
    void* f = base + ws.f;

    if (embed) {
        MEDP_TRY(medp_im2col_patch(pixels, a0, B, 3, H, W, w->patch, w->patch_kpad, stream));
        MEDP_TRY(medp_gemm_bf16_nt(a0, w->patch_w, patch, B * P, D, w->patch_kpad, w->patch_kpad, w->patch_kpad, D, w->patch_b,
                                   nullptr, nullptr, 0, 0, 0, stream));
        const float* pos_used = w->pos;
        if (!(gh == w->pos_side && gw == w->pos_side)) {
            MEDP_TRY(medp_pos_embed_bicubic(w->pos, pos, w->pos_side, gh, gw, D, stream));
            pos_used = pos;
        }
        MEDP_TRY(medp_vit_assemble(patch, w->cls, pos_used, x, B, P, D, stream));
    }
    const float scale = 0.125f;
    if (fold_wanted(w, M) && first_layer < last_layer) {
        bf16_t* xb = (bf16_t*)(base + ws.xb);
        float* stats = (float*)(base + ws.stats);
        const int NT = D / 256, Mpad = (M + 255) / 256 * 256;
        hipStream_t st = (hipStream_t)stream;
        if (NT == 1) rowstats_cast_kernel<1><<<(Mpad + 3) / 4, 256, 0, st>>>(x, xb, stats, M, Mpad, D);
        else if (NT == 2) rowstats_cast_kernel<2><<<(Mpad + 3) / 4, 256, 0, st>>>(x, xb, stats, M, Mpad, D);
        else if (NT == 3) rowstats_cast_kernel<3><<<(Mpad + 3) / 4, 256, 0, st>>>(x, xb, stats, M, Mpad, D);
        else rowstats_cast_kernel<4><<<(Mpad + 3) / 4, 256, 0, st>>>(x, xb, stats, M, Mpad, D);
        MEDP_LAUNCH_CHECK("vit rowstats_cast");
        MedpGemmFold cons{}, prod{};
        cons.stats_in = stats; cons.stats_tiles = NT; cons.ln_eps = w->ln_eps; cons.ln_dim = D;
        prod.c2 = xb; prod.ldc2 = D; prod.stats_out = stats;
        for (int l = first_layer; l < last_layer; ++l) {
            const MedpVitLayer& L = w->layers[l];
            cons.colsum = L.qkv_cs;
            MEDP_TRY(medp_gemm_bf16_nt_fold(xb, L.qkv_wg, qkv, M, 3 * D, D, D, D, 3 * D, L.qkv_b2, nullptr, nullptr, 0, 0, 1, cons, stream));
            MEDP_TRY(medp_attn_fwd_dh64(qkv, (const bf16_t*)qkv + D, (const bf16_t*)qkv + 2 * D, att, B, S, w->n_heads, 3 * D, 3 * D,
                                        3 * D, D, scale, stream));
            MEDP_TRY(medp_gemm_bf16_nt_fold(att, L.proj_w, x, M, D, D, D, D, D, L.proj_b, L.ls1, x, D, 0, 0, prod, stream));
            cons.colsum = L.fc1_cs;
            MEDP_TRY(medp_gemm_bf16_nt_fold(xb, L.fc1_wg, f, M, w->mlp_hidden, D, D, D, w->mlp_hidden, L.fc1_b2, nullptr, nullptr, 0, 1, 1, cons, stream));
            MEDP_TRY(medp_gemm_bf16_nt_fold(f, L.fc2_w, x, M, D, w->mlp_hidden, w->mlp_hidden, w->mlp_hidden, D, L.fc2_b, L.ls2, x, D, 0, 0, prod, stream));
        }
    } else {
        for (int l = first_layer; l < last_layer; ++l) {
            const MedpVitLayer& L = w->layers[l];
            MEDP_TRY(medp_layernorm_fwd(x, D, L.ln1_w, L.ln1_b, h, D, 1, nullptr, nullptr, M, D, w->ln_eps, stream));
            MEDP_TRY(medp_gemm_bf16_nt_tagged(1, h, L.qkv_w, qkv, M, 3 * D, D, D, D, 3 * D, L.qkv_b, nullptr, nullptr, 0, 0, 1, stream));
            MEDP_TRY(medp_attn_fwd_dh64(qkv, (const bf16_t*)qkv + D, (const bf16_t*)qkv + 2 * D, att, B, S, w->n_heads, 3 * D, 3 * D,
                                        3 * D, D, scale, stream));
            MEDP_TRY(medp_gemm_bf16_nt_tagged(1, att, L.proj_w, x, M, D, D, D, D, D, L.proj_b, L.ls1, x, D, 0, 0, stream));
            MEDP_TRY(medp_layernorm_fwd(x, D, L.ln2_w, L.ln2_b, h, D, 1, nullptr, nullptr, M, D, w->ln_eps, stream));
            MEDP_TRY(medp_gemm_bf16_nt_tagged(1, h, L.fc1_w, f, M, w->mlp_hidden, D, D, D, w->mlp_hidden, L.fc1_b, nullptr, nullptr, 0, 1, 1, stream));
            MEDP_TRY(medp_gemm_bf16_nt_tagged(1, f, L.fc2_w, x, M, D, w->mlp_hidden, w->mlp_hidden, w->mlp_hidden, D, L.fc2_b, L.ls2, x, D, 0, 0, stream));
        }
    }
    if (!finish) return 0;
    if (tokens_f32)
        MEDP_TRY(medp_layernorm_fwd(x, D, w->final_ln_w, w->final_ln_b, tokens_f32, D, 0, nullptr, nullptr, M, D, w->ln_eps, stream));
    if (tokens_bf16)
        MEDP_TRY(medp_layernorm_fwd(x, D, w->final_ln_w, w->final_ln_b, tokens_bf16, D, 1, nullptr, nullptr, M, D, w->ln_eps, stream));
    return 0;
}

extern "C" int medp_dbg_vit_lnfold(int on) {
    const int prev = g_vit_lnfold;
    g_vit_lnfold = on < 0 ? -1 : (on != 0);
    return prev;
}

extern "C" int medp_dbg_gemm_fold(const void* A, const void* W, void* C, int M, int N, int K, const float* bias, const float* scale,
                                  const float* residual, int act, int out_bf16, void* c2, float* stats_out, const float* stats_in,
                                  int stats_tiles, const float* colsum, float ln_eps, int ln_dim, void* stream) {
    MedpGemmFold f{};
    f.c2 = c2; f.ldc2 = N; f.stats_out = stats_out;
    f.stats_in = stats_in; f.stats_tiles = stats_tiles; f.colsum = colsum; f.ln_eps = ln_eps; f.ln_dim = ln_dim;
    return medp_gemm_bf16_nt_fold(A, W, C, M, N, K, K, K, N, bias, scale, residual, N, act, out_bf16, f, stream);
}
```

### multimodal_edema_prediction_amd/cxr.py

```python
from __future__ import annotations

import ctypes
from dataclasses import dataclass

import torch
import torch.nn as nn

from . import abi
from . import functional as Fn
from .abi import MedpVitLayer, MedpVitWeights, check, lib, ptr, stream


@dataclass
class Dinov2Cfg:
    hidden_size: int = 768
    num_hidden_layers: int = 12
    num_attention_heads: int = 12
    mlp_ratio: int = 4
    patch_size: int = 14
    image_size: int = 518
    layer_norm_eps: float = 1e-6
    layerscale_value: float = 1.0
    num_channels: int = 3


class _Node(nn.Module):
    """Plain container: lets us lay out nn.Parameters under exactly the reference's state_dict keys."""


def _set_param(root: nn.Module, key: str, value: nn.Parameter) -> None:
    parts = key.split(".")
    m = root
    for p in parts[:-1]:
        if not hasattr(m, p):
            m.add_module(p, _Node())
        m = getattr(m, p)
    m.register_parameter(parts[-1], value)


def dinov2_param_shapes(cfg: Dinov2Cfg) -> dict:
    D, ps, C = cfg.hidden_size, cfg.patch_size, cfg.num_channels
    n_pos = (cfg.image_size // ps) ** 2 + 1
    mlp = D * cfg.mlp_ratio
    sh = {"embeddings.cls_token": (1, 1, D), "embeddings.mask_token": (1, D),
          "embeddings.position_embeddings": (1, n_pos, D),
          "embeddings.patch_embeddings.projection.weight": (D, C, ps, ps),
          "embeddings.patch_embeddings.projection.bias": (D,)}
    for l in range(cfg.num_hidden_layers):
        p = f"encoder.layer.{l}."
        sh[p + "norm1.weight"] = (D,); sh[p + "norm1.bias"] = (D,)
        for n in ("query", "key", "value"):
            sh[p + f"attention.attention.{n}.weight"] = (D, D); sh[p + f"attention.attention.{n}.bias"] = (D,)
        sh[p + "attention.output.dense.weight"] = (D, D); sh[p + "attention.output.dense.bias"] = (D,)
        sh[p + "layer_scale1.lambda1"] = (D,)
        sh[p + "norm2.weight"] = (D,); sh[p + "norm2.bias"] = (D,)
        sh[p + "mlp.fc1.weight"] = (mlp, D); sh[p + "mlp.fc1.bias"] = (mlp,)
        sh[p + "mlp.fc2.weight"] = (D, mlp); sh[p + "mlp.fc2.bias"] = (D,)
        sh[p + "layer_scale2.lambda1"] = (D,)
    sh["layernorm.weight"] = (D,); sh["layernorm.bias"] = (D,)
    return sh


class Dinov2Backbone(nn.Module):

    def __init__(self, cfg: Dinov2Cfg | None = None):
        super().__init__()
        self.cfg = cfg or Dinov2Cfg()
        g = torch.Generator().manual_seed(0)
        for k, shape in dinov2_param_shapes(self.cfg).items():
            leaf = k.split(".")[-1]
            if leaf == "bias" or "mask_token" in k:
                v = torch.zeros(shape)
            elif leaf == "lambda1":
                v = torch.full(shape, float(self.cfg.layerscale_value))
            elif leaf == "weight" and len(shape) == 1:
                v = torch.ones(shape)
            else:
                v = torch.randn(shape, generator=g) * 0.02
            _set_param(self, k, nn.Parameter(v))
        self._prep = None
        self._prep_key = None
        self._ws = {}

    @property
    def config(self):
        return self.cfg

    def _prepare(self):
        sd = dict(self.named_parameters())
        key = tuple((p.data_ptr(), p._version) for p in sd.values())
        if self._prep is not None and self._prep_key == key:
            return self._prep
        c = self.cfg
        D = c.hidden_size
        dev = sd["layernorm.weight"].device
        keep = []

        def f32(t):
            t = t.detach().to(torch.float32).contiguous()
            keep.append(t)
            return t

        def bf(t2d):
            t = Fn.to_bf16(t2d.detach().to(torch.float32).contiguous())
            keep.append(t)
            return t

        K = c.num_channels * c.patch_size ** 2
        kpad = (K + 7) // 8 * 8
        pw = torch.zeros((D, kpad), dtype=torch.float32, device=dev)
        pw[:, :K] = sd["embeddings.patch_embeddings.projection.weight"].detach().reshape(D, K)
        layers = (MedpVitLayer * c.num_hidden_layers)()
        for l in range(c.num_hidden_layers):
            p = f"encoder.layer.{l}."
            L = layers[l]
            qkv_w = torch.cat([sd[p + f"attention.attention.{n}.weight"].detach() for n in ("query", "key", "value")], 0)
            qkv_b = torch.cat([sd[p + f"attention.attention.{n}.bias"].detach() for n in ("query", "key", "value")], 0)
            L.ln1_w, L.ln1_b = ptr(f32(sd[p + "norm1.weight"])), ptr(f32(sd[p + "norm1.bias"]))
            L.qkv_w, L.qkv_b = ptr(bf(qkv_w)), ptr(f32(qkv_b))
            L.proj_w, L.proj_b = ptr(bf(sd[p + "attention.output.dense.weight"])), ptr(f32(sd[p + "attention.output.dense.bias"]))
            L.ls1 = ptr(f32(sd[p + "layer_scale1.lambda1"]))
            L.ln2_w, L.ln2_b = ptr(f32(sd[p + "norm2.weight"])), ptr(f32(sd[p + "norm2.bias"]))
            L.fc1_w, L.fc1_b = ptr(bf(sd[p + "mlp.fc1.weight"])), ptr(f32(sd[p + "mlp.fc1.bias"]))
            L.fc2_w, L.fc2_b = ptr(bf(sd[p + "mlp.fc2.weight"])), ptr(f32(sd[p + "mlp.fc2.bias"]))
            L.ls2 = ptr(f32(sd[p + "layer_scale2.lambda1"]))
            for name, W, b, g, beta in (("qkv", qkv_w, qkv_b, sd[p + "norm1.weight"], sd[p + "norm1.bias"]),
                                        ("fc1", sd[p + "mlp.fc1.weight"], sd[p + "mlp.fc1.bias"], sd[p + "norm2.weight"], sd[p + "norm2.bias"])):
                W32 = W.detach().to(torch.float32)
                wg = bf(W32 * g.detach().to(torch.float32)[None, :])
                setattr(L, name + "_wg", ptr(wg))
                setattr(L, name + "_cs", ptr(f32(wg.to(torch.float32).sum(dim=1))))
                setattr(L, name + "_b2", ptr(f32(b.detach().to(torch.float32) + W32 @ beta.detach().to(torch.float32))))
        w = MedpVitWeights()
        w.hidden, w.n_layers, w.n_heads, w.mlp_hidden = D, c.num_hidden_layers, c.num_attention_heads, D * c.mlp_ratio
        w.patch, w.pos_side, w.patch_kpad, w.ln_eps = c.patch_size, c.image_size // c.patch_size, kpad, c.layer_norm_eps
        w.patch_w = ptr(bf(pw))
        w.patch_b = ptr(f32(sd["embeddings.patch_embeddings.projection.bias"]))
        w.cls = ptr(f32(sd["embeddings.cls_token"].reshape(-1)))
        w.pos = ptr(f32(sd["embeddings.position_embeddings"].reshape(-1, D)))
        w.final_ln_w, w.final_ln_b = ptr(f32(sd["layernorm.weight"])), ptr(f32(sd["layernorm.bias"]))
        w.layers = ctypes.cast(layers, ctypes.POINTER(MedpVitLayer))
        self._prep, self._prep_key = (w, layers, keep), key
        return self._prep

    def forward(self, pixel_values: torch.Tensor, want_f32: bool = True, want_bf16: bool = False, layers=None, slot: int = 0, out16=None):
        abi.require_gpu()
        if pixel_values.dim() != 4 or pixel_values.shape[1] != self.cfg.num_channels:
            raise ValueError("Make sure that the channel dimension of the pixel values match with the one set in the "
                             f"configuration. Expected {self.cfg.num_channels} but got {tuple(pixel_values.shape)}.")
        if any(p.requires_grad for p in self.parameters()) and torch.is_grad_enabled():
            from .cxr_train import forward_training
            if out16 is not None:
                raise ValueError("out16 is a frozen-path argument (the training path returns fp32 tokens with a gradient)")
            tok = forward_training(self, pixel_values)
            return (tok if want_f32 else None), (tok if want_bf16 else None)
        if Fn.precision() == "fp32" and layers is None:
            from .cxr_train import forward_fp32
            tok = forward_fp32(self, pixel_values)
            t16 = None
            if want_bf16:
                t16 = tok.to(torch.bfloat16) if out16 is None else out16.copy_(tok)
            return (tok if want_f32 else None), t16
        w, _, _ = self._prepare()
        px = pixel_values.detach().to(torch.float32).contiguous()
        B, _, H, W = px.shape
        P = (H // self.cfg.patch_size) * (W // self.cfg.patch_size)
        need = lib().medp_vit_workspace_bytes(ctypes.byref(w), B, H, W)
        ws = self._ws.get(slot)
        if ws is None or ws.numel() < need or ws.device != px.device:
            ws = self._ws[slot] = torch.empty(need, dtype=torch.uint8, device=px.device)
        D = self.cfg.hidden_size
        first, last = (0, self.cfg.num_hidden_layers) if layers is None else layers
        fin = last == self.cfg.num_hidden_layers
        out32 = torch.empty((B, P + 1, D), dtype=torch.float32, device=px.device) if (want_f32 and fin) else None
        if out16 is not None:
            if out16.shape != (B, P + 1, D) or out16.dtype != torch.bfloat16 or not out16.is_contiguous() or out16.device != px.device:
                raise ValueError("out16 must be a contiguous bf16 [B, P+1, hidden] tensor on the input's device")
        else:
            out16 = torch.empty((B, P + 1, D), dtype=torch.bfloat16, device=px.device) if (want_bf16 and fin) else None
        check(lib().medp_vit_forward_part(ctypes.byref(w), ptr(px), B, H, W, ptr(out32), ptr(out16), ptr(ws), need, first, last,
                                          stream()), "vit_forward")
        return out32, out16


class CXREncoder(nn.Module):

    def __init__(self, model_name: str = "microsoft/rad-dino", freeze: bool = True, return_patches: bool = True, *,
                 config: Dinov2Cfg | None = None):
        super().__init__()
        self.backbone = Dinov2Backbone(config)
        if config is None and model_name and model_name != "synthetic":
            self._try_load_pretrained(model_name)
        self.d_out = self.backbone.cfg.hidden_size
        self.return_patches = return_patches
        if freeze:
            for p in self.backbone.parameters():
                p.requires_grad = False
            self.backbone.eval()
        self._frozen = freeze

    def _try_load_pretrained(self, model_name: str) -> None:
        from transformers import AutoModel
        try:
            hf = AutoModel.from_pretrained(model_name, local_files_only=True)
        except Exception as e:
            raise RuntimeError(f"CXREncoder: pretrained weights for {model_name!r} are not available locally "
                               f"({type(e).__name__}: {e}); pass a local checkpoint directory, or model_name='synthetic' "
                               "for seeded random weights (synthetic benchmark only)") from e
        self.backbone.load_state_dict(hf.state_dict(), strict=True)

    def train(self, mode: bool = True):
        super().train(mode)
        if self._frozen:
            self.backbone.eval()
        return self

    def forward(self, pixel_values: torch.Tensor):
        tokens, _ = self.backbone(pixel_values)
        cls = tokens[:, 0]
        if self.return_patches:
            return cls, tokens[:, 1:]
        return cls

    def forward_bf16(self, pixel_values: torch.Tensor, slot: int = 0, out=None):
        if Fn.precision() == "fp32" and out is None and not (any(p.requires_grad for p in self.backbone.parameters()) and torch.is_grad_enabled()):
            return self.backbone(pixel_values, want_f32=True, want_bf16=False)[0]
        _, t16 = self.backbone(pixel_values, want_f32=False, want_bf16=True, slot=slot, out16=out)
        return t16

    def forward_bf16_part(self, pixel_values: torch.Tensor, first: int, last: int):
        if any(p.requires_grad for p in self.backbone.parameters()):
            raise RuntimeError("the encoder can only be run in pieces when it is frozen")
        _, t16 = self.backbone(pixel_values, want_f32=False, want_bf16=True, layers=(first, last))
        return t16
```

### multimodal_edema_prediction_amd/graph_step.py

```python
from __future__ import annotations

import os

import torch

from . import autograd_ops as _A, dp, engine
from .streams import new_stream, note_capture_origin
from .abi import check, lib, ptr, stream


def _stacked(v):
    return v if torch.is_tensor(v) else torch.stack(tuple(v))


class _TrainSnapshot:

    def __init__(self, modules, epoch, params=(), optimizer=None, extra=()):
        self.params, self.opt, self.modules, self.epoch = list(params), optimizer, list(modules), epoch
        with torch.no_grad():
            self.p = [q.detach().clone() for q in self.params]
            self.bufs = [(m, n, b.detach().clone()) for m in self.modules for n, b in m.named_buffers()]
            self.extra = [(t, t.detach().clone()) for t in extra]
            self.epoch0 = epoch.detach().clone()
            if optimizer is not None:
                self.state = {id(q): {k: (v.detach().clone() if torch.is_tensor(v) else v) for k, v in optimizer.state.get(q, {}).items()}
                              for q in self.params}
                self.host_step = optimizer._step

    def restore(self):
        with torch.no_grad():
            for q, v in zip(self.params, self.p):
                q.copy_(v)
            if self.params:
                torch.autograd.graph.increment_version(self.params)
            if self.opt is not None:
                for q in self.params:
                    st, old = self.opt.state.get(q, {}), self.state[id(q)]
                    for k, v in st.items():
                        if torch.is_tensor(v):
                            v.copy_(old[k]) if k in old else v.zero_()
                if self.opt.dev_step is not None:
                    self.opt.dev_step.fill_(self.host_step)
                self.opt._step = self.host_step
            for t, v in self.extra:
                t.copy_(v)
            for m, n, v in self.bufs:
                b = m.get_buffer(n)
                if not torch.equal(b, v):
                    b.copy_(v)
            self.epoch.copy_(self.epoch0)


_EPOCH_OWNER = [None]


def _register_epoch(epoch: torch.Tensor):
    check(lib().medp_rng_set_epoch_ptr(ptr(epoch)), "rng_set_epoch_ptr")
    _EPOCH_OWNER[0] = epoch


def _release_epoch(epoch: torch.Tensor):
    if _EPOCH_OWNER[0] is epoch:
        try:
            lib().medp_rng_set_epoch_ptr(None)
        finally:
            _EPOCH_OWNER[0] = None


class _CapturedStep:

    def __del__(self):
        ep = self.__dict__.get("epoch")
        if ep is not None:
            _release_epoch(ep)

    def _build(self, optimizer, device, warmup, before_capture):
        self.opt, self.device = optimizer, device
        self.params = [p for g in optimizer.param_groups for p in g["params"] if p.requires_grad]
        self.epoch = torch.zeros(1, dtype=torch.int32, device=device)
        _register_epoch(self.epoch)
        self._captured = False
        snap = _TrainSnapshot(self._stateful_modules(), self.epoch, self.params, optimizer)
        s = new_stream(device)
        s.wait_stream(torch.cuda.current_stream(device))
        n = max(int(warmup), 1)
        with torch.cuda.stream(s):
            for it in range(n):
                self._warmup_step(last=it == n - 1)
        torch.cuda.current_stream(device).wait_stream(s)
        torch.cuda.synchronize(device)
        self._zero_grads()
        snap.restore()
        torch.cuda.synchronize(device)
        if before_capture is not None:
            before_capture()
        self._streams_before_capture()
        self.g = torch.cuda.CUDAGraph()
        with torch.cuda.graph(self.g):
            note_capture_origin(device)
            self.out = self._captured_step()
        torch.cuda.synchronize(device)
        self._captured = True
        self.opt._step = int(self.opt.dev_step.item())
        self._prep_refs = [(m, m._prep) for root in self._stateful_modules() for m in root.modules() if getattr(m, "_prep", None) is not None]
        self._cache_refs = [v for slot in _A._W_CACHE.values() for v in slot.values()]
        self._keepalive = []
        for root in self._stateful_modules():
            for m in root.modules():
                ws = m.__dict__.get("_ws")
                self._keepalive += list(ws.values()) if isinstance(ws, dict) else ([ws] if torch.is_tensor(ws) else [])
                self._keepalive += list(m.__dict__.get("_tables", {}).values())

    def _warmup_step(self, last: bool):
        self._captured_step()

    def _zero_grads(self):
        self.opt.zero_grad(set_to_none=True)

    def _streams_before_capture(self):
        pass

    def _advance_epoch(self):
        check(lib().medp_counter_advance(ptr(self.epoch), stream()), "counter_advance")

    def _check_frozen_unchanged(self):
        for m, prep in self._prep_refs:
            if m._prep is not prep:
                raise RuntimeError(f"{type(m).__name__}: frozen weights were modified after the step was captured; build a new "
                                   f"{type(self).__name__} (the captured graph still reads the old prepared weights)")

    def _replay(self):
        self._check_frozen_unchanged()
        self.opt.refresh_lrs()
        self.g.replay()
        self._after_replay()
        return self.out

    def _after_replay(self):
        self.opt.note_external_step()


class _PipelinedStep(_CapturedStep):

    def _setup(self, optimizer, device, world, group, split, pipeline, warmup, before_capture, after_capture=None):
        self.world, self.group = world, group
        self.pipeline = bool(pipeline)
        self.split = bool(split) or world > 1
        self.arena = None
        self.force_collective = False
        self._pool = None
        self._expect = None
        self._staged, self.stage = None, None
        self.frozen_stream = new_stream(device) if self.pipeline else None
        self._build(optimizer, device, warmup, before_capture)
        if after_capture is not None:
            after_capture()
        self.phase_log = None
        if self.pipeline and os.environ.get("MEDP_PHASE_CHECK", "0") == "1":
            penalty, t_copy = self._staging_penalty()
            self.phase_log = (len(self._pad_streams), round(penalty * 1e3, 3), round(t_copy * 1e3, 3))

    def _streams_before_capture(self):
        self._pad_streams = [new_stream(self.device, raw=True) for _ in range(int(os.environ.get("MEDP_PRE_CAPTURE_STREAMS", str(self._default_pad_streams()))))]
        self.copy_stream = new_stream(self.device)

    def _default_pad_streams(self) -> int:
        return 3

    def _warmup_step(self, last: bool):
        if self.split and self.arena is None:
            snap = _TrainSnapshot(self._stateful_modules(), self.epoch)
            used = dp.find_used_parameters(self.params, lambda: (self._advance(), self._whole_fwd_bwd()))
            self.arena = dp.FlatGradArena(self.params, used=used, group=self.group)
            self.arena.bind(zero=True)
            snap.restore()
        self._zero_grads()
        self._advance()
        if last and os.environ.get("MEDP_OPERAND_POOL", "1") == "1":
            with _A.record_operands() as log:
                self._whole_fwd_bwd()
            self._pool = _A.WeightOperandPool(log, self.device)
        else:
            self._whole_fwd_bwd()
        self._allreduce()
        self.opt.step()

    def _captured_step(self):
        if not self.split:
            self._advance()
            return self._whole_fwd_bwd(then=self.opt.step)
        self.arena.flat.zero_()
        self._advance()
        return self._whole_fwd_bwd()

    def _staging_penalty(self, n: int = 6):
        import time
        dev_b, host_b = self._calib_batches()
        snap = _TrainSnapshot(self._stateful_modules(), self.epoch, self.params, self.opt, extra=self._handover_tensors())
        expect = self._expect

        def timed(pool, staged):
            ts = []
            for i in range(n + 3):
                torch.cuda.synchronize(self.device)
                t0 = time.perf_counter()
                self.step(pool[i % 2], pool[(i + 1) % 2], pool[i % 2] if staged else None)
                torch.cuda.synchronize(self.device)
                ts.append(time.perf_counter() - t0)
            return sorted(ts[3:])[n // 2]

        t_res, t_host = timed(dev_b, False), timed(host_b, True)
        px = host_b[0]["pixel_values"]
        dst = torch.empty_like(dev_b[0]["pixel_values"])
        torch.cuda.synchronize(self.device)
        t0 = time.perf_counter()
        with torch.cuda.stream(self.copy_stream):
            for _ in range(n):
                dst.copy_(px, non_blocking=True)
        torch.cuda.synchronize(self.device)
        t_copy = (time.perf_counter() - t0) / n
        snap.restore()
        self._expect, self._staged = expect, None
        torch.cuda.synchronize(self.device)
        penalty = t_host - t_res
        if self.world > 1:
            pt = torch.tensor([penalty, t_copy], device=self.device, dtype=torch.float64)
            torch.distributed.all_reduce(pt, op=torch.distributed.ReduceOp.MAX, group=self.group)
            penalty, t_copy = float(pt[0]), float(pt[1])
        return penalty, t_copy

    def _zero_grads(self):
        if self.arena is None:
            self.opt.zero_grad(set_to_none=True)
        else:
            self.arena.bind(zero=True)

    def _advance(self):
        self._advance_epoch()
        if self._pool is not None:
            self._pool.refresh()

    def _allreduce(self):
        if self.arena is not None and (self.world > 1 or self.force_collective):
            self.arena.all_reduce(force=self.force_collective)

    def _whole_fwd_bwd(self, then=None):
        if not self.pipeline:
            out = self._train_fwd_bwd()
            if then is not None:
                then()
            return out
        cur = torch.cuda.current_stream(self.device)
        self.frozen_stream.wait_stream(cur)
        with torch.cuda.stream(self.frozen_stream):
            self._frozen_forward()
        out = self._train_fwd_bwd()
        if then is not None:
            then()
        cur.wait_stream(self.frozen_stream)
        self._hand_over()
        return out

    def _after_replay(self):
        if not self.split:
            return super()._after_replay()
        ring = self._split_events()
        ring[0].record()
        self._allreduce()
        ring[1].record()
        self.opt.relaunch()
        ring[2].record()

    def _split_events(self):
        if not hasattr(self, "_sev"):
            self._sev = [[torch.cuda.Event(enable_timing=True) for _ in range(3)] for _ in range(64)]
            self._sev_n = 0
        ev = self._sev[self._sev_n % 64]
        self._sev_n += 1
        return ev

    def split_timings(self):
        n = min(getattr(self, "_sev_n", 0), 64)
        if n == 0:
            return None
        torch.cuda.synchronize(self.device)
        ar = sum(e[0].elapsed_time(e[1]) for e in self._sev[:n]) / n
        up = sum(e[1].elapsed_time(e[2]) for e in self._sev[:n]) / n
        return {"allreduce_ms": round(ar, 4), "optimizer_ms": round(up, 4), "steps": n,
                "collective": "one mean all-reduce of the flat fp32 gradient arena between the forward/backward graph and the optimiser launches"}

    def _stage(self, next_batch: dict, after_next: dict) -> None:
        if self.stage is None:
            self.stage = {k: torch.empty_like(v) for k, v in self._stage_buffers().items()}
            self.h2d_done, self.stage_free = torch.cuda.Event(), torch.cuda.Event()
            self.stage_free.record(torch.cuda.current_stream(self.device))
        with torch.cuda.stream(self.copy_stream):
            self.copy_stream.wait_event(self.stage_free)
            self._stage_h2d(next_batch, after_next)
            self.h2d_done.record(self.copy_stream)
        self._staged = (next_batch, after_next)

    def step(self, batch: dict | None = None, next_batch: dict | None = None, after_next: dict | None = None) -> dict:
        st = self._staged
        staged = self.pipeline and batch is not None and next_batch is not None and st is not None and st[0] is batch and st[1] is next_batch
        if batch is not None and self.pipeline and self._expect is not batch:
            self.prime(batch)
        if staged:
            cur = torch.cuda.current_stream(self.device)
            cur.wait_event(self.h2d_done)
            self._take_staged()
            self.stage_free.record(cur)
            self._expect = next_batch
        else:
            if batch is not None:
                self.load_batch(batch)
            nb = next_batch if next_batch is not None else batch
            if self.pipeline and nb is not None:
                self._load_next(nb)
                self._expect = nb
        if self.pipeline and after_next is not None and next_batch is not None and not next_batch["pixel_values"].is_cuda:
            self._stage(next_batch, after_next)
        else:
            self._staged = None
        return self._replay()


class GraphedTeacherStep(_PipelinedStep):
    def __init__(self, teacher, loss_fn, optimizer, example_batch: dict, device, world: int = 1, group=None, warmup: int = 3,
                 split: bool = False, before_capture=None, pipeline_cxr: bool = False, after_capture=None):
        self.teacher, self.loss_fn = teacher, loss_fn
        b = engine._move_lists(example_batch, device)
        self.x_ts = torch.stack(b["x_ts"]).contiguous()
        self.x_static = torch.stack(b["x_static"]).contiguous()
        self.bin_ends = torch.stack(b["bin_ends"]).contiguous()
        self.pixels = b["pixel_values"].clone()
        if pipeline_cxr:
            if any(p.requires_grad for p in teacher.cxr.parameters()):
                raise ValueError("pipeline_cxr needs a frozen CXR encoder")
            self.pixels_next = self.pixels.clone()
            with torch.no_grad():
                self.tok_cur = teacher.cxr.forward_bf16(self.pixels).clone()
            self.tok_next = torch.empty_like(self.tok_cur)
        self.y_multi = b["y_multi"].clone().float()
        self.y_mask = b["y_multi_mask"].clone().float()
        engine._set_train_with_frozen_eval(teacher)
        self._setup(optimizer, device, world, group, split, pipeline_cxr, warmup, before_capture, after_capture)

    def _frozen_forward(self):
        with torch.no_grad():
            self.teacher.cxr.forward_bf16(self.pixels_next, out=self.tok_next)

    def _stateful_modules(self):
        return [self.teacher]

    def _handover_tensors(self):
        return [self.tok_cur] if self.pipeline else []

    def _small_buffers(self):
        return {"x_ts": self.x_ts, "x_static": self.x_static, "bin_ends": self.bin_ends, "y_multi": self.y_multi, "y_multi_mask": self.y_mask}

    def _calib_batches(self):
        d = {k: v.clone() for k, v in dict(self._small_buffers(), pixel_values=self.pixels).items()}
        h = {k: v.cpu().pin_memory() for k, v in d.items()}
        return [dict(d), dict(d)], [dict(h), dict(h)]

    def _hand_over(self):
        self.tok_cur.copy_(self.tok_next)

    def _train_fwd_bwd(self):
        B = self.x_ts.shape[0]
        out = self.teacher(tuple(self.x_ts[i] for i in range(B)), tuple(self.x_static[i] for i in range(B)),
                           tuple(self.bin_ends[i] for i in range(B)), self.pixels,
                           **({"_cxr_tokens16": self.tok_cur} if self.pipeline else {}))
        losses = self.loss_fn(out["img_logits"], out["ts_logits"], out["fusion_logits"], self.y_multi, self.y_mask)
        losses["total"].backward()
        return {"loss": losses["total"].detach(), "img_total": losses["img_total"], "ts_total": losses["ts_total"],
                "fus_total": losses["fus_total"], "fusion_logits": out["fusion_logits"].detach(), "main_logit": out["main_logit"].detach()}

    def prime(self, batch: dict) -> None:
        with torch.no_grad():
            self.tok_cur.copy_(self.teacher.cxr.forward_bf16(batch["pixel_values"].to(self.device, non_blocking=True)))
        self._expect = batch

    def load_batch(self, batch: dict) -> None:
        for k, buf in self._small_buffers().items():
            buf.copy_(_stacked(batch[k]), non_blocking=True)
        if not self.pipeline:
            self.pixels.copy_(batch["pixel_values"], non_blocking=True)

    def _load_next(self, batch: dict) -> None:
        self.pixels_next.copy_(batch["pixel_values"], non_blocking=True)

    def _stage_buffers(self):
        return dict(self._small_buffers(), pixel_values=self.pixels_next)

    def _stage_h2d(self, next_batch: dict, after_next: dict) -> None:
        for k in self._small_buffers():
            self.stage[k].copy_(_stacked(next_batch[k]), non_blocking=True)
        self.stage["pixel_values"].copy_(after_next["pixel_values"], non_blocking=True)

    def _take_staged(self) -> None:
        for k, buf in self._stage_buffers().items():
            buf.copy_(self.stage[k])


class GraphedStudentStep(_PipelinedStep):

    def __init__(self, student, teacher, kd_loss_fn, optimizer, example_batch: dict, device, world: int = 1, group=None,
                 warmup: int = 3, split: bool = False, before_capture=None, pipeline_teacher: bool = True, after_capture=None,
                 swap_roles=None):
        if any(p.requires_grad for p in teacher.parameters()):
            raise ValueError("the KD teacher must be frozen (trainer.py:856-865)")
        self.student, self.teacher, self.loss_fn = student, teacher, kd_loss_fn
        import inspect
        self._teacher_kw = set(inspect.signature(teacher.forward).parameters)
        b = engine._move_lists(example_batch, device)
        mk = lambda: {"x_ts": torch.stack(b["x_ts"]).contiguous(), "x_static": torch.stack(b["x_static"]).contiguous(),
                      "bin_ends": torch.stack(b["bin_ends"]).contiguous(), "pixel_values": b["pixel_values"].clone()}
        self.cur = mk()
        self.nxt = mk() if pipeline_teacher else None
        self.y = b["y"].clone().float()
        student.train()
        teacher.eval()
        with torch.no_grad():
            self.z_cur = self._teacher_logit(self.cur).clone()
        self.z_next = None
        self.swap_roles = (os.environ.get("MEDP_STUDENT_SWAP", "1") == "1") if swap_roles is None else bool(swap_roles)
        self._setup(optimizer, device, world, group, split, pipeline_teacher, warmup, before_capture, after_capture)

    def _default_pad_streams(self) -> int:
        return 1 if self.swap_roles else 3

    def _teacher_logit(self, bufs, forked: bool = False):
        B = bufs["x_ts"].shape[0]
        kw = {"_overlap": False} if (forked and "_overlap" in self._teacher_kw) else {}
        return self.teacher(tuple(bufs["x_ts"][i] for i in range(B)), tuple(bufs["x_static"][i] for i in range(B)),
                            tuple(bufs["bin_ends"][i] for i in range(B)), bufs["pixel_values"], **kw)["main_logit"]

    def _frozen_forward(self):
        with torch.no_grad():
            self.z_next = self._teacher_logit(self.nxt, forked=not self.swap_roles)

    def _whole_fwd_bwd(self, then=None):
        if not (self.pipeline and self.swap_roles):
            return super()._whole_fwd_bwd(then)
        cur = torch.cuda.current_stream(self.device)
        ts = self.frozen_stream
        ts.wait_stream(cur)
        with torch.cuda.stream(ts):
            out = self._train_fwd_bwd()
            if then is not None:
                then()
        self._frozen_forward()
        cur.wait_stream(ts)
        self._hand_over()
        return out

    def _stateful_modules(self):
        return [self.student, self.teacher]

    def _handover_tensors(self):
        return [self.z_cur]

    def _calib_batches(self):
        d = {k: v.clone() for k, v in self.cur.items()}
        d["y"] = self.y.clone()
        h = {k: v.cpu().pin_memory() for k, v in d.items()}
        return [dict(d), dict(d)], [dict(h), dict(h)]

    def _hand_over(self):
        if not self._captured:
            self.z_next.record_stream(torch.cuda.current_stream(self.device))
        self.z_cur.copy_(self.z_next)

    def _train_fwd_bwd(self):
        if not self.pipeline:
            with torch.no_grad():
                self.z_cur.copy_(self._teacher_logit(self.cur))
        B = self.cur["x_ts"].shape[0]
        z_s = self.student(tuple(self.cur["x_ts"][i] for i in range(B)), tuple(self.cur["x_static"][i] for i in range(B)),
                           tuple(self.cur["bin_ends"][i] for i in range(B)))
        losses = self.loss_fn(z_s, self.z_cur, self.y)
        losses["total"].backward()
        return {"loss": losses["total"].detach(), "bce": losses["bce"], "kd": losses["kd"], "logits": z_s.detach()}

    @staticmethod
    def _load(bufs, batch, with_pixels=True):
        bufs["x_ts"].copy_(_stacked(batch["x_ts"]), non_blocking=True)
        bufs["x_static"].copy_(_stacked(batch["x_static"]), non_blocking=True)
        bufs["bin_ends"].copy_(_stacked(batch["bin_ends"]), non_blocking=True)
        if with_pixels:
            bufs["pixel_values"].copy_(batch["pixel_values"], non_blocking=True)

    def prime(self, batch: dict) -> None:
        self._load(self.nxt, batch)
        with torch.no_grad():
            self.z_cur.copy_(self._teacher_logit(self.nxt))
        self._expect = batch

    def load_batch(self, batch: dict) -> None:
        self._load(self.cur, batch, with_pixels=not self.pipeline)
        self.y.copy_(batch["y"], non_blocking=True)

    def _load_next(self, batch: dict) -> None:
        self._load(self.nxt, batch)

    def _stage_buffers(self):
        return dict(self.nxt, y=self.y)

    def _stage_h2d(self, next_batch: dict, after_next: dict) -> None:
        self._load(self.stage, after_next)
        self.stage["y"].copy_(next_batch["y"], non_blocking=True)

    def _take_staged(self) -> None:
        for k in ("x_ts", "x_static", "bin_ends"):
            self.cur[k].copy_(self.nxt[k])
        self.y.copy_(self.stage["y"])
        for k, v in self.nxt.items():
            v.copy_(self.stage[k])


class _GraphedProbe(_CapturedStep):

    def __init__(self, probe, loss_fn, optimizer, x, y, mask, device, warmup, before_capture):
        self.probe, self.loss_fn = probe, loss_fn
        self.x = x.to(device).clone()
        self.y = y.to(device).float().clone()
        self.mask = mask.to(device).float().clone()
        self._build(optimizer, device, warmup, before_capture)

    def _stateful_modules(self):
        return [self.probe]

    def _captured_step(self):
        self._advance_epoch()
        self.opt.zero_grad(set_to_none=True)
        loss = self.loss_fn(self.probe(self.x), self.y, self.mask)
        loss.backward()
        self.opt.step()
        return {"loss": loss.detach()}

    def _copy_and_replay(self, x, y, mask) -> dict:
        if x is not None and x.data_ptr() != self.x.data_ptr():
            self.x.copy_(x, non_blocking=True)
        if y is not None:
            self.y.copy_(y, non_blocking=True)
            self.mask.copy_(mask, non_blocking=True)
        return self._replay()


class GraphedProbeStep(_GraphedProbe):

    def __init__(self, probe, loss_fn, optimizer, example_pixels, example_y, example_mask, device, warmup: int = 3, before_capture=None):
        super().__init__(probe, loss_fn, optimizer, example_pixels, example_y, example_mask, device, warmup, before_capture)

    def step(self, pixel_values=None, y_multi=None, y_multi_mask=None) -> dict:
        return self._copy_and_replay(pixel_values, y_multi, y_multi_mask)


class GraphedTrajectoryProbeStep(_GraphedProbe):

    def __init__(self, probe, loss_fn, optimizer, example_x, example_y, example_mask, device, warmup: int = 3, before_capture=None):
        super().__init__(probe, loss_fn, optimizer, _stacked(example_x).float(), example_y, example_mask, device, warmup, before_capture)

    def step(self, x_ts=None, y=None, mask=None) -> dict:
        return self._copy_and_replay(None if x_ts is None else _stacked(x_ts), y, mask)
```

Measured before the change: 12980.

## Batch device copies, fuse im2col with class rows, cache pos table, add rowmap GEMM

Adds a multi-job copy kernel so the several per-batch device-to-device buffer copies run as one launch instead of many. Adds a strip-based im2col kernel that stages each patch row in LDS and also writes the class-token rows, which removes a separate assembly launch. Caches the bicubic-resized position table when the weights are frozen, and adds a rowmap GEMM variant that adds the positional residual and writes into the shifted token rows directly. These cut launch count and intermediate traffic, at the cost of more code paths and stale-cache risk if the weights change.

```diff
diff --git a/include/medp_hip.h b/include/medp_hip.h
--- a/include/medp_hip.h
+++ b/include/medp_hip.h
@@ -99,6 +99,13 @@
 } MedpOperandJob;
 int medp_weight_operands_multi(const MedpOperandJob* dev_jobs, const int* dev_block_job, const int* dev_block_tile, int n_blocks,
                                void* stream);
+#define MEDP_COPY_MAX_JOBS 8
+typedef struct {
+    void* dst;
+    const void* src;
+    size_t bytes;
+} MedpCopyJob;
+int medp_copy_multi(const MedpCopyJob* host_jobs, int n_jobs, void* stream);
 int medp_gelu_bwd(const float* dy, const float* pre, float* dx, long long n, void* stream);
 int medp_gelu_bf16_fwd(const void* pre, void* out, long long n, void* stream);
 int medp_gelu_bf16_bwd(const void* dy, const void* pre, void* dx, long long n, void* stream);
@@ -129,6 +136,8 @@
     const float *patch_b, *cls, *pos;
     const float *final_ln_w, *final_ln_b;
     const MedpVitLayer* layers;
+    const float* pos_table;
+    int pos_gh, pos_gw;
 } MedpVitWeights;
 
 size_t medp_vit_workspace_bytes(const MedpVitWeights* host_w, int B, int H, int W);
diff --git a/multimodal_edema_prediction_amd/abi.py b/multimodal_edema_prediction_amd/abi.py
--- a/multimodal_edema_prediction_amd/abi.py
+++ b/multimodal_edema_prediction_amd/abi.py
@@ -22,7 +22,8 @@
     _fields_ = ([(n, I) for n in ("hidden", "n_layers", "n_heads", "mlp_hidden", "patch", "pos_side", "patch_kpad")]
                 + [("ln_eps", F)]
                 + [(n, P) for n in ("patch_w", "patch_b", "cls", "pos", "final_ln_w", "final_ln_b")]
-                + [("layers", ctypes.POINTER(MedpVitLayer))])
+                + [("layers", ctypes.POINTER(MedpVitLayer))]
+                + [("pos_table", P), ("pos_gh", I), ("pos_gw", I)])
 
 
 class MedpEncoderWeights(ctypes.Structure):
@@ -47,6 +48,13 @@
 class MedpOperandJob(ctypes.Structure):
     _fields_ = [("src", P), ("dst_plain", P), ("dst_t", P), ("rows", I), ("cols", I), ("ld_src", I), ("ld_plain", I), ("ld_t", I),
                 ("reserved_", I)]
+
+
+class MedpCopyJob(ctypes.Structure):
+    _fields_ = [("dst", P), ("src", P), ("bytes", SZ)]
+
+
+COPY_MAX_JOBS = 8
 
 
 SIGNATURES = {
@@ -88,6 +96,7 @@
     "medp_cast_f32_bf16": (I, [P, I, P, I, I, I, P]),
     "medp_transpose_to_bf16": (I, [P, I, I, P, I, I, I, P]),
     "medp_weight_operands_multi": (I, [P, P, P, I, P]),
+    "medp_copy_multi": (I, [ctypes.POINTER(MedpCopyJob), I, P]),
     "medp_gelu_bwd": (I, [P, P, P, LL, P]),
     "medp_gelu_bf16_fwd": (I, [P, P, LL, P]),
     "medp_gelu_bf16_bwd": (I, [P, P, P, LL, P]),
diff --git a/multimodal_edema_prediction_amd/csrc/api.cpp b/multimodal_edema_prediction_amd/csrc/api.cpp
--- a/multimodal_edema_prediction_amd/csrc/api.cpp
+++ b/multimodal_edema_prediction_amd/csrc/api.cpp
@@ -13,7 +13,7 @@
 }
 
 extern "C" const char* medp_last_error(void) { return g_err; }
-extern "C" int medp_version(void) { return 2; }
+extern "C" int medp_version(void) { return 3; }
 extern "C" const char* medp_arch(void) { return "gfx950"; }
 
 #include <stdint.h>
diff --git a/multimodal_edema_prediction_amd/csrc/elementwise.hip b/multimodal_edema_prediction_amd/csrc/elementwise.hip
--- a/multimodal_edema_prediction_amd/csrc/elementwise.hip
+++ b/multimodal_edema_prediction_amd/csrc/elementwise.hip
@@ -105,6 +105,59 @@
     }
 }
 
+__device__ __forceinline__ void vit_class_rows(const float* __restrict__ cls, const float* __restrict__ pos, float* __restrict__ x,
+                                               int B, int S, int D, unsigned first, unsigned stride) {
+    const unsigned d4 = D >> 2, total = (unsigned)B * d4;
+    for (unsigned i = first; i < total; i += stride) {
+        const unsigned b = i / d4, c = (i - b * d4) * 4;
+        const float4 v = *(const float4*)(cls + c), pe = *(const float4*)(pos + c);
+        *(float4*)(x + (size_t)b * S * D + c) = make_float4(v.x + pe.x, v.y + pe.y, v.z + pe.z, v.w + pe.w);
+    }
+}
+__global__ __launch_bounds__(256) void vit_class_rows_kernel(const float* __restrict__ cls, const float* __restrict__ pos,
+                                                             float* __restrict__ x, int B, int S, int D) {
+    vit_class_rows(cls, pos, x, B, S, D, blockIdx.x * 256u + threadIdx.x, gridDim.x * 256u);
+}
+template <int PS>
+__global__ __launch_bounds__(256) void im2col_strip_kernel(const float* __restrict__ pix, bf16_t* __restrict__ A, int B, int C, int H, int W,
+                                                           int ps_rt, int kpad, int nstrips, const float* __restrict__ cls,
+                                                           const float* __restrict__ pos, float* __restrict__ x, int D) {
+    extern __shared__ __attribute__((aligned(16))) char strip_lds[];
+    const unsigned ps = PS ? PS : ps_rt;
+    const unsigned gh = H / ps, gw = W / ps, K = C * ps * ps, pp = ps * ps;
+    if ((int)blockIdx.x >= nstrips) {
+        vit_class_rows(cls, pos, x, B, (int)(gh * gw) + 1, D, (blockIdx.x - nstrips) * 256u + threadIdx.x, (gridDim.x - nstrips) * 256u);
+        return;
+    }
+    const unsigned b = blockIdx.x / gh, py = blockIdx.x - b * gh;
+    uint32_t* lds = (uint32_t*)strip_lds;
+    const unsigned kp2 = kpad >> 1, npad2 = (kpad - K) >> 1;
+    for (unsigned i = threadIdx.x; i < gw * npad2; i += 256) {
+        const unsigned px = i / npad2;
+        lds[px * kp2 + (K >> 1) + (i - px * npad2)] = 0u;
+    }
+    const unsigned w4 = W >> 2, wuse = gw * ps, nrows = C * ps;
+    const float* img = pix + (size_t)b * C * H * W + (size_t)(py * ps) * W;
+    for (unsigned i = threadIdx.x; i < nrows * w4; i += 256) {
+        const unsigned r = i / w4, col = (i - r * w4) * 4;
+        if (col >= wuse) continue;
+        const unsigned c = r / ps, ii = r - c * ps;
+        const float4 v = *(const float4*)(img + ((size_t)c * H + ii) * W + col);
+        const unsigned kb = c * pp + ii * ps;
+        const unsigned px0 = col / ps, j0 = col - px0 * ps;
+        lds[px0 * kp2 + ((kb + j0) >> 1)] = pack_bf2(v.x, v.y);
+        const unsigned col1 = col + 2;
+        if (col1 < wuse) {
+            const unsigned px1 = col1 / ps, j1 = col1 - px1 * ps;
+            lds[px1 * kp2 + ((kb + j1) >> 1)] = pack_bf2(v.z, v.w);
+        }
+    }
+    __syncthreads();
+    const unsigned n16 = gw * (kpad >> 3);
+    uint4* dst = (uint4*)(A + (size_t)blockIdx.x * gw * kpad);
+    for (unsigned i = threadIdx.x; i < n16; i += 256) dst[i] = ((const uint4*)strip_lds)[i];
+}
+
 __global__ __launch_bounds__(256) void im2col_patch_kernel(const float* __restrict__ pix, bf16_t* __restrict__ A, int B, int C, int H,
                                                            int W, int ps, int kpad) {
     const unsigned gh = H / ps, gw = W / ps, K = C * ps * ps, pp = ps * ps, k8 = kpad >> 3;
@@ -219,6 +272,23 @@
     }
 }
 
+struct CopyJobs {
+    MedpCopyJob j[MEDP_COPY_MAX_JOBS];
+};
+__global__ __launch_bounds__(256) void copy_multi_kernel(const CopyJobs jobs) {
+    const MedpCopyJob jb = jobs.j[blockIdx.y];
+    char* dst = (char*)jb.dst;
+    const char* src = (const char*)jb.src;
+    const size_t n = jb.bytes, first = (size_t)blockIdx.x * 256 + threadIdx.x, stride = (size_t)gridDim.x * 256;
+    size_t done = 0;
+    if ((((uintptr_t)dst | (uintptr_t)src) & 15) == 0) {
+        const size_t n16 = n >> 4;
+        for (size_t i = first; i < n16; i += stride) ((uint4*)dst)[i] = ((const uint4*)src)[i];
+        done = n16 << 4;
+    }
+    for (size_t i = done + first; i < n; i += stride) dst[i] = src[i];
+}
+
 inline int grid_for(size_t work_items) { return (int)min((size_t)4096, max((size_t)1, (work_items + 255) / 256)); }
 
 }
@@ -272,14 +342,55 @@
     return 0;
 }
 
-extern "C" int medp_im2col_patch(const float* pix, void* A, int B, int C, int H, int W, int patch, int kpad, void* stream) {
+int medp_im2col_patch_cls(const float* pix, void* A, int B, int C, int H, int W, int patch, int kpad, const float* cls, const float* pos,
+                          float* x, int D, void* stream) {
     MEDP_CHECK_ARG(pix && A && B > 0 && C > 0 && patch > 0, "im2col: bad argument");
     MEDP_CHECK_ARG(H >= patch && W >= patch, "im2col: image %dx%d smaller than the patch size %d", H, W, patch);
     MEDP_CHECK_ARG(kpad >= C * patch * patch && kpad % 8 == 0, "im2col: kpad must be >= C*p*p and a multiple of 8");
-    const size_t total = (size_t)B * (H / patch) * (W / patch) * (kpad / 8);
+    MEDP_CHECK_ARG(!x || (cls && pos && D > 0 && D % 4 == 0), "im2col: class rows need cls, pos and D % 4 == 0");
+    const int gh = H / patch, gw = W / patch;
+    const size_t total = (size_t)B * gh * gw * (kpad / 8);
     MEDP_CHECK_ARG(total < (1ull << 31), "im2col: B * patches * kpad / 8 must stay below 2^31");
-    im2col_patch_kernel<<<grid_for(total), 256, 0, (hipStream_t)stream>>>(pix, (bf16_t*)A, B, C, H, W, patch, kpad);
+    MEDP_CHECK_ARG(!x || (size_t)B * D / 4 < (1ull << 31), "im2col: B * D / 4 must stay below 2^31");
+    hipStream_t st = (hipStream_t)stream;
+    static const int strip_on = [] { const char* e = getenv("MEDP_IM2COL_STRIP"); return e ? atoi(e) : 1; }();
+    const size_t lds = (size_t)gw * kpad * 2;
+    if (strip_on && patch % 2 == 0 && W % 4 == 0 && ((uintptr_t)pix & 15) == 0 && ((uintptr_t)A & 15) == 0 && lds <= 64 * 1024 &&
+        (size_t)B * gh < (1u << 30)) {
+        const int nstrips = B * gh, ncls = x ? (int)min((size_t)256, ((size_t)B * D / 4 + 255) / 256) : 0;
+        if (patch == 14)
+            im2col_strip_kernel<14><<<nstrips + ncls, 256, lds, st>>>(pix, (bf16_t*)A, B, C, H, W, patch, kpad, nstrips, cls, pos, x, D);
+        else
+            im2col_strip_kernel<0><<<nstrips + ncls, 256, lds, st>>>(pix, (bf16_t*)A, B, C, H, W, patch, kpad, nstrips, cls, pos, x, D);
+        MEDP_LAUNCH_CHECK("medp_im2col_patch(strip)");
+        return 0;
+    }
+    im2col_patch_kernel<<<grid_for(total), 256, 0, st>>>(pix, (bf16_t*)A, B, C, H, W, patch, kpad);
     MEDP_LAUNCH_CHECK("medp_im2col_patch");
+    if (x) {
+        vit_class_rows_kernel<<<grid_for((size_t)B * D / 4), 256, 0, st>>>(cls, pos, x, B, gh * gw + 1, D);
+        MEDP_LAUNCH_CHECK("medp_im2col_patch(class rows)");
+    }
+    return 0;
+}
+
+extern "C" int medp_im2col_patch(const float* pix, void* A, int B, int C, int H, int W, int patch, int kpad, void* stream) {
+    return medp_im2col_patch_cls(pix, A, B, C, H, W, patch, kpad, nullptr, nullptr, nullptr, 0, stream);
+}
+
+extern "C" int medp_copy_multi(const MedpCopyJob* host_jobs, int n_jobs, void* stream) {
+    MEDP_CHECK_ARG(host_jobs && n_jobs > 0 && n_jobs <= MEDP_COPY_MAX_JOBS, "copy_multi: 1..%d jobs", MEDP_COPY_MAX_JOBS);
+    CopyJobs jobs{};
+    size_t most = 0;
+    for (int i = 0; i < n_jobs; ++i) {
+        MEDP_CHECK_ARG(host_jobs[i].bytes == 0 || (host_jobs[i].dst && host_jobs[i].src), "copy_multi: job %d has a null pointer", i);
+        jobs.j[i] = host_jobs[i];
+        most = max(most, host_jobs[i].bytes);
+    }
+    if (most == 0) return 0;
+    const int gx = (int)min((size_t)1024, (most / 16 + 255) / 256 + 1);
+    copy_multi_kernel<<<dim3(gx, n_jobs), 256, 0, (hipStream_t)stream>>>(jobs);
+    MEDP_LAUNCH_CHECK("medp_copy_multi");
     return 0;
 }
 
diff --git a/multimodal_edema_prediction_amd/csrc/gemm_bf16.hip b/multimodal_edema_prediction_amd/csrc/gemm_bf16.hip
--- a/multimodal_edema_prediction_amd/csrc/gemm_bf16.hip
+++ b/multimodal_edema_prediction_amd/csrc/gemm_bf16.hip
@@ -472,6 +472,29 @@
                    "gemm(fold): a consumer needs colsum, ln_dim, 1..4 stats tiles, a bf16 result and no residual / scale");
     MEDP_CHECK_ARG(!fold.c2 || (fold.stats_out && !out_bf16 && fold.ldc2 % 4 == 0), "gemm(fold): a producer writes fp32 C, c2 (ld % 4 == 0) and stats_out");
     return gemm_dispatch(1, A, W, C, M, N, K, lda, ldw, ldc, bias, scale, residual, ldr, act, out_bf16, nullptr, 0, &fold, stream);
+}
+
+bool medp_gemm_rowmap_eligible(int M, int N, int K, int period) {
+    static const int force = [] { const char* e = getenv("MEDP_GEMM_VARIANT"); return e ? atoi(e) : 0; }();
+    static const int v7_on = [] { const char* e = getenv("MEDP_GEMM_V7"); return e ? atoi(e) : 1; }();
+    if (period < 4 || M <= 0 || M % period != 0 || N <= 64 || N % 4 != 0 || K % 8 != 0 || !uses_tile256(M, N)) return false;
+    if ((long long)(M / period) * (period + 1) > 0x7fffffffLL / 2) return false;
+    MedpGemmArgs a{};
+    a.M = M; a.N = N; a.K = K;
+    return !(force != 6 && v7_on && medp_gemm_v7_eligible(a));
+}
+
+int medp_gemm_bf16_nt_rowmap(const void* A, const void* W, float* C, int M, int N, int K, int lda, int ldw, int ldc, const float* bias,
+                             const float* residual, int ldr, int period, void* stream) {
+    MEDP_CHECK_ARG(A && W && C && residual, "gemm(rowmap): null operand");
+    MEDP_CHECK_ARG(medp_gemm_rowmap_eligible(M, N, K, period), "gemm(rowmap): M=%d N=%d K=%d period=%d does not take the v6 kernel", M, N, K, period);
+    MEDP_CHECK_ARG(lda % 8 == 0 && ldw % 8 == 0 && lda >= K && ldw >= K && ldc % 4 == 0 && ldc >= N && ldr % 4 == 0 && ldr >= N,
+                   "gemm(rowmap): bad leading dimension");
+    MEDP_CHECK_ARG(((uintptr_t)A & 15) == 0 && ((uintptr_t)W & 15) == 0 && ((uintptr_t)C & 15) == 0 && ((uintptr_t)residual & 15) == 0 &&
+                   (!bias || ((uintptr_t)bias & 15) == 0), "gemm(rowmap): operands must be 16-byte aligned");
+    MedpGemmArgs a{A, W, C, M, N, K, lda, ldw, ldc, bias, nullptr, residual, ldr, 0, 0, nullptr, 0};
+    a.rowmap_period = period;
+    return medp_gemm_v6_launch(a, 0, stream);
 }
 
 int medp_gemm_bf16_nt_tagged(int tag, const void* A, const void* W, void* C, int M, int N, int K, int lda, int ldw, int ldc,
diff --git a/multimodal_edema_prediction_amd/csrc/gemm_bf16_v6.hip b/multimodal_edema_prediction_amd/csrc/gemm_bf16_v6.hip
--- a/multimodal_edema_prediction_amd/csrc/gemm_bf16_v6.hip
+++ b/multimodal_edema_prediction_amd/csrc/gemm_bf16_v6.hip
@@ -16,6 +16,7 @@
     static_assert(GR == 128 || GR == 112, "v6 group rows");
     constexpr int BM = 2 * GR;
     constexpr int NI1 = (GR - 64) / 16;
+    constexpr bool RM = TAG == 2;
     extern __shared__ __attribute__((aligned(16))) char smem[];
     const int tid = threadIdx.x, lane = tid & 63;
     const int wave = __builtin_amdgcn_readfirstlane(tid >> 6);
@@ -142,11 +143,24 @@
         if (p.scale) scale4 = *(const f32x4*)(p.scale + n);
     }
     f32x4 res[2][16];
+    const int rm_period = RM ? p.rowmap_period : 1;
     auto load_res = [&](int half) {
-#pragma unroll
-        for (int it = 0; it < 16; ++it) {
-            const int m = m0 + wm * GR + half * 64 + it * 4 + er;
-            res[half][it] = (half * 64 + it * 4 < GR && m < p.M && n < p.N) ? *(const f32x4*)(p.residual + (size_t)m * p.ldr + n) : (f32x4){0.f, 0.f, 0.f, 0.f};
+        if constexpr (RM) {
+            const int mf = m0 + wm * GR + half * 64 + er;
+            int pr = mf % rm_period;
+#pragma unroll
+            for (int it = 0; it < 16; ++it) {
+                const int m = mf + it * 4;
+                res[half][it] = (half * 64 + it * 4 < GR && m < p.M && n < p.N) ? *(const f32x4*)(p.residual + (size_t)(pr + 1) * p.ldr + n) : (f32x4){0.f, 0.f, 0.f, 0.f};
+                pr += 4;
+                if (pr >= rm_period) pr -= rm_period;
+            }
+        } else {
+#pragma unroll
+            for (int it = 0; it < 16; ++it) {
+                const int m = m0 + wm * GR + half * 64 + it * 4 + er;
+                res[half][it] = (half * 64 + it * 4 < GR && m < p.M && n < p.N) ? *(const f32x4*)(p.residual + (size_t)m * p.ldr + n) : (f32x4){0.f, 0.f, 0.f, 0.f};
+            }
         }
     };
     const bool has_res = p.residual != nullptr;
@@ -165,6 +179,12 @@
             for (int j = 0; j < 4; ++j) *(f32x4*)(wl + (i4 * 16 + fr) * 68 + j * 16 + kq * 4) = acc[half * 4 + i4][j];
         MEDP_WAVE_LDS_SYNC();
         if (half == 0 && has_res) load_res(1);
+        int crow = 0, cpr = 0;
+        if constexpr (RM) {
+            const int mf = m0 + wm * GR + half * 64 + er, img = mf / rm_period;
+            cpr = mf - img * rm_period;
+            crow = mf + img + 1;
+        }
 #pragma unroll
         for (int it = 0; it < 16; ++it) {
             if (half * 64 + it * 4 >= GR) continue;
@@ -194,9 +214,9 @@
                     o.x = pack_bf2(v[0], v[1]);
                     o.y = pack_bf2(v[2], v[3]);
                     typedef __attribute__((ext_vector_type(2))) unsigned int u32x2;
-                    __builtin_nontemporal_store((u32x2){o.x, o.y}, (u32x2*)((bf16_t*)p.C + (size_t)m * p.ldc + n));
+                    __builtin_nontemporal_store((u32x2){o.x, o.y}, (u32x2*)((bf16_t*)p.C + (size_t)(RM ? crow : m) * p.ldc + n));
                 } else {
-                    __builtin_nontemporal_store(v, (f32x4*)((float*)p.C + (size_t)m * p.ldc + n));
+                    __builtin_nontemporal_store(v, (f32x4*)((float*)p.C + (size_t)(RM ? crow : m) * p.ldc + n));
                 }
                 if (producer) {
                     uint2 o;
@@ -218,6 +238,11 @@
                 s1 = row16_sum(s1);
                 s2 = row16_sum(s2);
                 if ((lane & 15) == 0) *(float2*)(sst + ((wm * 128 + half * 64 + rr) * 4 + wn) * 2) = make_float2(s1, s2);
+            }
+            if constexpr (RM) {
+                cpr += 4;
+                crow += 4;
+                if (cpr >= rm_period) { cpr -= rm_period; ++crow; }
             }
         }
         MEDP_WAVE_LDS_SYNC();
@@ -267,8 +292,20 @@
 
 }
 
+namespace {
+int g_rowmap_launches = 0, g_rowmap_tile_rows = 0;
+}
+extern "C" int medp_dbg_gemm_rowmap_launches(void) { return g_rowmap_launches; }
+extern "C" int medp_dbg_gemm_rowmap_last_tile_rows(void) { return g_rowmap_tile_rows; }
+
 int medp_gemm_v6_launch(const MedpGemmArgs& a, int tag, void* stream) {
     hipStream_t s = (hipStream_t)stream;
+    if (a.rowmap_period > 0) {
+        const bool t224 = v6_use_224(a);
+        ++g_rowmap_launches;
+        g_rowmap_tile_rows = t224 ? 224 : 256;
+        return t224 ? launch_v6_gr<2, 112>(a, s) : launch_v6_gr<2, 128>(a, s);
+    }
     if (v6_use_224(a)) return tag == 1 ? launch_v6_gr<1, 112>(a, s) : launch_v6_gr<0, 112>(a, s);
     return tag == 1 ? launch_v6_gr<1, 128>(a, s) : launch_v6_gr<0, 128>(a, s);
 }
diff --git a/multimodal_edema_prediction_amd/csrc/gemm_variants.h b/multimodal_edema_prediction_amd/csrc/gemm_variants.h
--- a/multimodal_edema_prediction_amd/csrc/gemm_variants.h
+++ b/multimodal_edema_prediction_amd/csrc/gemm_variants.h
@@ -20,6 +20,7 @@
     int ldr, act, out_bf16;
     unsigned long long* prof;
     int prof_flags;
+    int rowmap_period = 0;
     MedpGemmFold fold;
 };
 #define MEDP_PROF_ENTER(prof, flags)                                                                                       \
@@ -41,6 +42,9 @@
         }                                                                                                                  \
     } while (0)
 int medp_gemm_v6_launch(const MedpGemmArgs& a, int tag, void* stream);
+bool medp_gemm_rowmap_eligible(int M, int N, int K, int period);
+int medp_gemm_bf16_nt_rowmap(const void* A, const void* W, float* C, int M, int N, int K, int lda, int ldw, int ldc, const float* bias,
+                             const float* residual, int ldr, int period, void* stream);
 int medp_gemm_ragged_rows_launch(const MedpGemmArgs& a, int m_begin, void* stream);
 bool medp_gemm_v7_eligible(const MedpGemmArgs& a);
 unsigned* medp_gemm_ticket_block(void* stream);
diff --git a/multimodal_edema_prediction_amd/csrc/vit.hip b/multimodal_edema_prediction_amd/csrc/vit.hip
--- a/multimodal_edema_prediction_amd/csrc/vit.hip
+++ b/multimodal_edema_prediction_amd/csrc/vit.hip
@@ -3,6 +3,9 @@
 #include "common.h"
 #include "gemm_variants.h"
 #include "medp_hip.h"
+
+int medp_im2col_patch_cls(const float* pix, void* A, int B, int C, int H, int W, int patch, int kpad, const float* cls, const float* pos,
+                          float* x, int D, void* stream);
 
 namespace {
 inline size_t al(size_t x) { return (x + 255) & ~(size_t)255; }
@@ -52,6 +55,12 @@
     s.stats = off; off += al(((M + 255) / 256 * 256) * (D / 256 + 1) * 2 * 4);
     s.total = off;
     return s;
+}
+
+int g_vit_embed_fused = -1;
+bool embed_fused_wanted() {
+    static const int env_on = [] { const char* e = getenv("MEDP_VIT_EMBED_FUSED"); return e ? atoi(e) : 1; }();
+    return (g_vit_embed_fused >= 0 ? g_vit_embed_fused : env_on) != 0;
 }
 
 int g_vit_lnfold = -1;
@@ -104,15 +113,25 @@
     void* f = base + ws.f;
 
     if (embed) {
-        MEDP_TRY(medp_im2col_patch(pixels, a0, B, 3, H, W, w->patch, w->patch_kpad, stream));
-        MEDP_TRY(medp_gemm_bf16_nt(a0, w->patch_w, patch, B * P, D, w->patch_kpad, w->patch_kpad, w->patch_kpad, D, w->patch_b,
-                                   nullptr, nullptr, 0, 0, 0, stream));
         const float* pos_used = w->pos;
         if (!(gh == w->pos_side && gw == w->pos_side)) {
-            MEDP_TRY(medp_pos_embed_bicubic(w->pos, pos, w->pos_side, gh, gw, D, stream));
-            pos_used = pos;
-        }
-        MEDP_TRY(medp_vit_assemble(patch, w->cls, pos_used, x, B, P, D, stream));
+            if (w->pos_table && w->pos_gh == gh && w->pos_gw == gw) {
+                pos_used = w->pos_table;
+            } else {
+                MEDP_TRY(medp_pos_embed_bicubic(w->pos, pos, w->pos_side, gh, gw, D, stream));
+                pos_used = pos;
+            }
+        }
+        if (embed_fused_wanted() && D % 4 == 0 && medp_gemm_rowmap_eligible(B * P, D, w->patch_kpad, P)) {
+            MEDP_TRY(medp_im2col_patch_cls(pixels, a0, B, 3, H, W, w->patch, w->patch_kpad, w->cls, pos_used, x, D, stream));
+            MEDP_TRY(medp_gemm_bf16_nt_rowmap(a0, w->patch_w, x, B * P, D, w->patch_kpad, w->patch_kpad, w->patch_kpad, D, w->patch_b,
+                                              pos_used, D, P, stream));
+        } else {
+            MEDP_TRY(medp_im2col_patch(pixels, a0, B, 3, H, W, w->patch, w->patch_kpad, stream));
+            MEDP_TRY(medp_gemm_bf16_nt(a0, w->patch_w, patch, B * P, D, w->patch_kpad, w->patch_kpad, w->patch_kpad, D, w->patch_b,
+                                       nullptr, nullptr, 0, 0, 0, stream));
+            MEDP_TRY(medp_vit_assemble(patch, w->cls, pos_used, x, B, P, D, stream));
+        }
     }
     const float scale = 0.125f;
     if (fold_wanted(w, M) && first_layer < last_layer) {
@@ -160,6 +179,12 @@
     return 0;
 }
 
+extern "C" int medp_dbg_vit_embed_fused(int on) {
+    const int prev = g_vit_embed_fused;
+    g_vit_embed_fused = on < 0 ? -1 : (on != 0);
+    return prev;
+}
+
 extern "C" int medp_dbg_vit_lnfold(int on) {
     const int prev = g_vit_lnfold;
     g_vit_lnfold = on < 0 ? -1 : (on != 0);
diff --git a/multimodal_edema_prediction_amd/cxr.py b/multimodal_edema_prediction_amd/cxr.py
--- a/multimodal_edema_prediction_amd/cxr.py
+++ b/multimodal_edema_prediction_amd/cxr.py
@@ -1,6 +1,7 @@
 from __future__ import annotations
 
 import ctypes
+import os
 from dataclasses import dataclass
 
 import torch
@@ -22,6 +23,9 @@
     layer_norm_eps: float = 1e-6
     layerscale_value: float = 1.0
     num_channels: int = 3
+
+
+_POS_CACHE = os.environ.get("MEDP_POS_CACHE", "1") != "0"
 
 
 class _Node(nn.Module):
@@ -140,8 +144,20 @@
         w.pos = ptr(f32(sd["embeddings.position_embeddings"].reshape(-1, D)))
         w.final_ln_w, w.final_ln_b = ptr(f32(sd["layernorm.weight"])), ptr(f32(sd["layernorm.bias"]))
         w.layers = ctypes.cast(layers, ctypes.POINTER(MedpVitLayer))
-        self._prep, self._prep_key = (w, layers, keep), key
+        self._prep, self._prep_key = (w, layers, keep, {}), key
         return self._prep
+
+    def _pos_table(self, prep, gh: int, gw: int):
+        w, _, _, tables = prep
+        if not _POS_CACHE or (gh == w.pos_side and gw == w.pos_side) or any(p.requires_grad for p in self.parameters()):
+            return None
+        t = tables.get((gh, gw))
+        if t is None:
+            pos = self.embeddings.position_embeddings
+            t = torch.empty((gh * gw + 1, w.hidden), dtype=torch.float32, device=pos.device)
+            check(lib().medp_pos_embed_bicubic(w.pos, ptr(t), w.pos_side, gh, gw, w.hidden, stream()), "pos_embed_bicubic")
+            tables[(gh, gw)] = t
+        return t
 
     def forward(self, pixel_values: torch.Tensor, want_f32: bool = True, want_bf16: bool = False, layers=None, slot: int = 0, out16=None):
         abi.require_gpu()
@@ -161,9 +177,12 @@
             if want_bf16:
                 t16 = tok.to(torch.bfloat16) if out16 is None else out16.copy_(tok)
             return (tok if want_f32 else None), t16
-        w, _, _ = self._prepare()
+        prep = self._prepare()
+        w = prep[0]
         px = pixel_values.detach().to(torch.float32).contiguous()
         B, _, H, W = px.shape
+        table = self._pos_table(prep, H // self.cfg.patch_size, W // self.cfg.patch_size)
+        w.pos_table, w.pos_gh, w.pos_gw = (ptr(table), H // self.cfg.patch_size, W // self.cfg.patch_size) if table is not None else (None, 0, 0)
         P = (H // self.cfg.patch_size) * (W // self.cfg.patch_size)
         need = lib().medp_vit_workspace_bytes(ctypes.byref(w), B, H, W)
         ws = self._ws.get(slot)
diff --git a/multimodal_edema_prediction_amd/graph_step.py b/multimodal_edema_prediction_amd/graph_step.py
--- a/multimodal_edema_prediction_amd/graph_step.py
+++ b/multimodal_edema_prediction_amd/graph_step.py
@@ -6,7 +6,22 @@
 
 from . import autograd_ops as _A, dp, engine
 from .streams import new_stream, note_capture_origin
-from .abi import check, lib, ptr, stream
+from .abi import COPY_MAX_JOBS, MedpCopyJob, check, lib, ptr, stream
+
+_BATCH_LOAD = os.environ.get("MEDP_BATCH_LOAD", "1") != "0"
+
+
+def _copy_many(pairs) -> None:
+    pairs = list(pairs)
+    if not (_BATCH_LOAD and len(pairs) > 1 and all(s.is_cuda and s.device == d.device and s.dtype == d.dtype and s.shape == d.shape
+                                                  and s.is_contiguous() and d.is_contiguous() for d, s in pairs)):
+        for d, s in pairs:
+            d.copy_(s, non_blocking=True)
+        return
+    for i in range(0, len(pairs), COPY_MAX_JOBS):
+        chunk = pairs[i:i + COPY_MAX_JOBS]
+        jobs = (MedpCopyJob * len(chunk))(*[MedpCopyJob(d.data_ptr(), s.data_ptr(), d.numel() * d.element_size()) for d, s in chunk])
+        check(lib().medp_copy_multi(jobs, len(chunk), stream()), "copy_multi")
 
 
 def _stacked(v):
@@ -312,12 +327,12 @@
             self.stage_free.record(cur)
             self._expect = next_batch
         else:
-            if batch is not None:
-                self.load_batch(batch)
+            pairs = self._batch_pairs(batch) if batch is not None else []
             nb = next_batch if next_batch is not None else batch
             if self.pipeline and nb is not None:
-                self._load_next(nb)
+                pairs += self._next_pairs(nb)
                 self._expect = nb
+            _copy_many(pairs)
         if self.pipeline and after_next is not None and next_batch is not None and not next_batch["pixel_values"].is_cuda:
             self._stage(next_batch, after_next)
         else:
@@ -382,14 +397,20 @@
             self.tok_cur.copy_(self.teacher.cxr.forward_bf16(batch["pixel_values"].to(self.device, non_blocking=True)))
         self._expect = batch
 
+    def _batch_pairs(self, batch: dict) -> list:
+        pairs = [(buf, _stacked(batch[k])) for k, buf in self._small_buffers().items()]
+        if not self.pipeline:
+            pairs.append((self.pixels, batch["pixel_values"]))
+        return pairs
+
+    def _next_pairs(self, batch: dict) -> list:
+        return [(self.pixels_next, batch["pixel_values"])]
+
     def load_batch(self, batch: dict) -> None:
-        for k, buf in self._small_buffers().items():
-            buf.copy_(_stacked(batch[k]), non_blocking=True)
-        if not self.pipeline:
-            self.pixels.copy_(batch["pixel_values"], non_blocking=True)
+        _copy_many(self._batch_pairs(batch))
 
     def _load_next(self, batch: dict) -> None:
-        self.pixels_next.copy_(batch["pixel_values"], non_blocking=True)
+        _copy_many(self._next_pairs(batch))
 
     def _stage_buffers(self):
         return dict(self._small_buffers(), pixel_values=self.pixels_next)
@@ -400,8 +421,7 @@
         self.stage["pixel_values"].copy_(after_next["pixel_values"], non_blocking=True)
 
     def _take_staged(self) -> None:
-        for k, buf in self._stage_buffers().items():
-            buf.copy_(self.stage[k])
+        _copy_many([(buf, self.stage[k]) for k, buf in self._stage_buffers().items()])
 
 
 class GraphedStudentStep(_PipelinedStep):
@@ -485,12 +505,15 @@
         return {"loss": losses["total"].detach(), "bce": losses["bce"], "kd": losses["kd"], "logits": z_s.detach()}
 
     @staticmethod
-    def _load(bufs, batch, with_pixels=True):
-        bufs["x_ts"].copy_(_stacked(batch["x_ts"]), non_blocking=True)
-        bufs["x_static"].copy_(_stacked(batch["x_static"]), non_blocking=True)
-        bufs["bin_ends"].copy_(_stacked(batch["bin_ends"]), non_blocking=True)
+    def _pairs(bufs, batch, with_pixels=True) -> list:
+        pairs = [(bufs[k], _stacked(batch[k])) for k in ("x_ts", "x_static", "bin_ends")]
         if with_pixels:
-            bufs["pixel_values"].copy_(batch["pixel_values"], non_blocking=True)
+            pairs.append((bufs["pixel_values"], batch["pixel_values"]))
+        return pairs
+
+    @classmethod
+    def _load(cls, bufs, batch, with_pixels=True):
+        _copy_many(cls._pairs(bufs, batch, with_pixels))
 
     def prime(self, batch: dict) -> None:
         self._load(self.nxt, batch)
@@ -498,12 +521,17 @@
             self.z_cur.copy_(self._teacher_logit(self.nxt))
         self._expect = batch
 
+    def _batch_pairs(self, batch: dict) -> list:
+        return self._pairs(self.cur, batch, with_pixels=not self.pipeline) + [(self.y, batch["y"])]
+
+    def _next_pairs(self, batch: dict) -> list:
+        return self._pairs(self.nxt, batch)
+
     def load_batch(self, batch: dict) -> None:
-        self._load(self.cur, batch, with_pixels=not self.pipeline)
-        self.y.copy_(batch["y"], non_blocking=True)
+        _copy_many(self._batch_pairs(batch))
 
     def _load_next(self, batch: dict) -> None:
-        self._load(self.nxt, batch)
+        _copy_many(self._next_pairs(batch))
 
     def _stage_buffers(self):
         return dict(self.nxt, y=self.y)
@@ -513,11 +541,8 @@
         self.stage["y"].copy_(next_batch["y"], non_blocking=True)
 
     def _take_staged(self) -> None:
-        for k in ("x_ts", "x_static", "bin_ends"):
-            self.cur[k].copy_(self.nxt[k])
-        self.y.copy_(self.stage["y"])
-        for k, v in self.nxt.items():
-            v.copy_(self.stage[k])
+        _copy_many([(self.cur[k], self.nxt[k]) for k in ("x_ts", "x_static", "bin_ends")] + [(self.y, self.stage["y"])])
+        _copy_many([(v, self.stage[k]) for k, v in self.nxt.items()])
 
 
 class _GraphedProbe(_CapturedStep):
```

Measured after the change: 13060, median of 6. About the same (+0.6%).
